# rizar/attention-lvcsr

Measured on NVIDIA H100. Metric: encoder+decoder frames/sec at batch64x1000frx40fb, higher is better.
Workload: dtype f32

## Files before the change

attention-lvcsr_b200/_lib.py:

```python
import ctypes as C
import os

_HERE = os.path.dirname(os.path.abspath(__file__))
LIB_PATH = os.environ.get("LVSR_B200_LIB") or os.path.join(_HERE, "csrc", "liblvsr_b200.so")

LVSR_MAX_LAYERS = 8
NORMALIZERS = {"softmax": 0, "logistic": 1, "relu": 2}
ACTIVATIONS = {"maxout": 0, "relu": 1, "tanh": 2, "identity": 3}
PRIORS = {"expanding": 0, "window_around_mean": 1, "window_around_median": 2}
ATTENTION_TYPES = {"content_and_conv": 0, "content": 1}
PLAN_SLOTS = ("ran", "kernel", "cs", "grid", "nisl", "nrg", "ncg", "nc1", "nc2", "nc3", "tc_cap", "wh_rows", "red_alias",
              "att_cs", "max_clusters")
PLAN_KERNELS = ("stepwise", "dec_scan", "dec_scan<COMPACT>", "dec_content")
ENC_PLAN_SLOTS = ("proj", "kpad", "bigru", "tape", "rb", "cs", "clusters", "resident", "waves", "T", "bwd_cs", "wgrad",
                  "wgrad_splits", "wgrad_kpad", "dx")
ENC_PATHS = (None, "tc", "ffma")
ENC_BIGRU_KERNELS = (None, "ffma", "mma")


class LvsrConfig(C.Structure):
    _fields_ = [
        ("num_features", C.c_int32),
        ("num_layers", C.c_int32),
        ("dims_bidir", C.c_int32 * LVSR_MAX_LAYERS),
        ("subsample", C.c_int32 * LVSR_MAX_LAYERS),
        ("dim_dec", C.c_int32),
        ("dim_matcher", C.c_int32),
        ("conv_n", C.c_int32),
        ("conv_num_filters", C.c_int32),
        ("num_phonemes", C.c_int32),
        ("dim_feedback", C.c_int32),
        ("post_merge_dim", C.c_int32),
        ("maxout_pieces", C.c_int32),
        ("post_merge_activation", C.c_int32),
        ("use_states_for_readout", C.c_int32),
        ("energy_normalizer", C.c_int32),
        ("prior_type", C.c_int32),
        ("prior_initial_begin", C.c_double),
        ("prior_initial_end", C.c_double),
        ("prior_min_speed", C.c_double),
        ("prior_max_speed", C.c_double),
        ("prior_before", C.c_double),
        ("prior_after", C.c_double),
        ("one_of_n_feedback", C.c_int32),
        ("attention_type", C.c_int32),
    ]


class LvsrTrainConfig(C.Structure):
    _fields_ = [("gradient_threshold", C.c_float), ("use_momentum", C.c_int32), ("scale", C.c_float),
                ("momentum", C.c_float), ("use_adadelta", C.c_int32), ("decay_rate", C.c_float),
                ("epsilon", C.c_float), ("max_norm", C.c_float), ("burn_in_steps", C.c_int32), ("decay", C.c_float)]


LM_MAX_STATES = 7


class LvsrLmFusion(C.Structure):
    _fields_ = [("weight", C.c_double), ("am_beta", C.c_double), ("no_transition_cost", C.c_double),
                ("normalize_am_weights", C.c_int32), ("normalize_lm_weights", C.c_int32),
                ("normalize_tot_weights", C.c_int32)]


_P = C.c_void_p
_I = C.c_int32
VALIDATE_FN = C.CFUNCTYPE(C.c_int32, _P, C.c_int32, C.POINTER(C.c_int64), C.c_int32)
SIGNATURES = {
    "lvsr_last_error": (C.c_char_p, []),
    "lvsr_version": (C.c_int, []),
    "lvsr_model_create": (C.c_int, [C.POINTER(LvsrConfig), C.POINTER(_P)]),
    "lvsr_model_destroy": (C.c_int, [_P]),
    "lvsr_model_num_params": (C.c_int, [_P]),
    "lvsr_model_param_name": (C.c_char_p, [_P, C.c_int]),
    "lvsr_model_param_shape": (C.c_int, [_P, C.c_int, C.POINTER(C.c_int64), C.POINTER(C.c_int32)]),
    "lvsr_model_set_param": (C.c_int, [_P, C.c_char_p, _P, C.c_int64]),
    "lvsr_model_get_param": (C.c_int, [_P, C.c_char_p, _P, C.c_int64]),
    "lvsr_model_flat_size": (C.c_int64, [_P]),
    "lvsr_model_param_offset": (C.c_int, [_P, C.c_int, C.POINTER(C.c_int64), C.POINTER(C.c_int64)]),
    "lvsr_model_flat_params": (C.c_void_p, [_P]),
    "lvsr_model_finalize": (C.c_int, [_P]),
    "lvsr_model_status": (C.c_int, [_P, C.POINTER(C.c_int32), C.POINTER(C.c_int64)]),
    "lvsr_model_decoder_plan": (C.c_int, [_P, C.POINTER(C.c_int32)]),
    "lvsr_model_encoder_plan": (C.c_int, [_P, _I, C.POINTER(C.c_int32)]),
    "lvsr_encoded_length": (C.c_int, [_P, _I]),
    "lvsr_encoded_dim": (C.c_int, [_P]),
    "lvsr_encoder_forward": (C.c_int, [_P, _P, _P, _I, _I, _P, _P, _P]),
    "lvsr_preprocess": (C.c_int, [_P, _P, _I, _I, _P, _P]),
    "lvsr_cost_matrix": (C.c_int, [_P, _P, _P, _I, _I, _P, _P, _I, _P, _P, _P, _P, _P, _P]),
    "lvsr_initial_states": (C.c_int, [_P, _I, _I, _P, _P, _P, _P, _P, _P, _P]),
    "lvsr_logprobs": (C.c_int, [_P, _P, _P, _P, _I, _I, _P, _I, _P, _P, _P, _P, _P]),
    "lvsr_next_states": (C.c_int, [_P, _P, _P, _P, _I, _I, _P, _I, _P, _P, _P, _P, _P, _P, _P, _P, _P, _P]),
    "lvsr_beam_search_many": (C.c_int, [_P, _P, _P, _P, _I, _I, _P, _P, _I, _I, _I, C.c_double, C.c_double, _I, VALIDATE_FN,
                                        _P, C.POINTER(_P), _P]),
    "lvsr_search_result_count": (C.c_int, [_P, _I]),
    "lvsr_search_result_length": (C.c_int, [_P, _I, _I]),
    "lvsr_search_result_get": (C.c_int, [_P, _I, _I, _P, _P]),
    "lvsr_search_result_destroy": (C.c_int, [_P]),
    "lvsr_model_set_lm": (C.c_int, [_P, _I, _I, _P, C.c_int64, _P, _P, _P, C.POINTER(LvsrLmFusion)]),
    "lvsr_model_clear_lm": (C.c_int, [_P]),
    "lvsr_lm_initial_states": (C.c_int, [_P, _I, _P, _P, _P, _P]),
    "lvsr_lm_next_states": (C.c_int, [_P, _I, _P, _P, _P, _P, _P, _P, _P]),
    "lvsr_recognizer_cost_host": (C.c_int, [_P, _P, _P, _P, _P, _I, _I, _I, _P, _P]),
    "lvsr_train_cost_and_grads": (C.c_int, [_P, _P, _P, _P, _P, _I, _I, _I, C.c_float, _P, _P, _P]),
    "lvsr_train_apply_updates": (C.c_int, [_P, _P, C.c_float, C.POINTER(LvsrTrainConfig), _P]),
    "lvsr_train_gradient_norm": (C.c_int, [_P, C.POINTER(C.c_float)]),
    "lvsr_train_reset": (C.c_int, [_P]),
    "lvsr_launch_count": (C.c_int64, [C.c_int]),
    "lvsr_profile_enable": (C.c_int, [C.c_int]),
    "lvsr_profile_read": (C.c_int, [C.c_char_p, C.POINTER(C.c_double), C.POINTER(C.c_int64)]),
}

_lib = None


def load():
    global _lib
    if _lib is not None:
        return _lib
    if not os.path.exists(LIB_PATH):
        raise RuntimeError(
            "%s is missing: build it with `python -c 'import __graft_entry__ as g; g.build()'` "
            "(attention-lvcsr_b200 has no CPU or PyTorch fallback)" % LIB_PATH)
    lib = C.CDLL(LIB_PATH)
    for name, (res, args) in SIGNATURES.items():
        fn = getattr(lib, name)
        fn.restype = res
        fn.argtypes = args
    _lib = lib
    return lib


def check(rc):
    if rc != 0:
        msg = load().lvsr_last_error()
        raise RuntimeError("lvsr_b200: " + (msg.decode("utf-8", "replace") if msg else "error %d" % rc))
```

attention-lvcsr_b200/csrc/api.cu:

```cuda
#include "lvsr_b200.h"

#include <stdarg.h>
#include <stdlib.h>

#include <algorithm>
#include <map>
#include <string>
#include <vector>

#include "model.h"

namespace lvsr {

thread_local std::string g_last_error;
long long g_launch_count = 0;

int set_error(const char* fmt, ...) {
  char buf[1024];
  va_list ap;
  va_start(ap, fmt);
  vsnprintf(buf, sizeof(buf), fmt, ap);
  va_end(ap);
  g_last_error = buf;
  return 1;
}

struct ProfEntry { std::string cls; cudaEvent_t a, b; };
static bool g_prof_on = false;
static std::vector<ProfEntry> g_prof;

ProfScope::ProfScope(const char* kernel_class, cudaStream_t stream) : slot(-1), st(stream) {
  if (!g_prof_on) return;
  ProfEntry e;
  e.cls = kernel_class;
  if (cudaEventCreate(&e.a) != cudaSuccess || cudaEventCreate(&e.b) != cudaSuccess) return;
  cudaEventRecord(e.a, st);
  g_prof.push_back(e);
  slot = (int)g_prof.size() - 1;
}
ProfScope::~ProfScope() {
  if (slot >= 0) cudaEventRecord(g_prof[slot].b, st);
}

}

using namespace lvsr;

namespace lvsr {

void add_param(lvsr_model* m, const std::string& name, int64_t d0, int64_t d1 = -1) {
  Param p;
  p.name = name;
  p.shape[0] = d0;
  p.shape[1] = d1 > 0 ? d1 : 1;
  p.ndim = d1 > 0 ? 2 : 1;
  p.count = d0 * (d1 > 0 ? d1 : 1);
  p.dev = nullptr;
  m->index[name] = (int)m->params.size();
  m->params.push_back(p);
}


void build_param_table(lvsr_model* m) {
  const lvsr_config& c = m->cfg;
  int din = c.num_features;
  for (int l = 0; l < c.num_layers; ++l) {
    const int D = c.dims_bidir[l];
    for (int dir = 0; dir < 2; ++dir) {
      const std::string b = enc_base(l, dir);
      add_param(m, b + "/gatedrecurrent.state_to_state", D, D);
      add_param(m, b + "/gatedrecurrent.state_to_gates", D, 2 * D);
      add_param(m, b + "/gatedrecurrent.initial_state", D);
      add_param(m, b + "/fork/fork_inputs.b", D);
      add_param(m, b + "/fork/fork_inputs.W", din, D);
      add_param(m, b + "/fork/fork_gate_inputs.b", 2 * D);
      add_param(m, b + "/fork/fork_gate_inputs.W", din, 2 * D);
    }
    din = 2 * D;
  }
  const int E = m->E, C = c.dim_dec, M = c.dim_matcher, K = c.conv_num_filters, w = 2 * c.conv_n + 1;
  const int V = c.num_phonemes, Cfb = c.dim_feedback, Cpm = c.post_merge_dim;
  const std::string g = GEN, t = TR, a = att_base(m);
  if (!c.one_of_n_feedback) add_param(m, g + "/readout/lookupfeedback/lookuptable.W", V + 1, Cfb);
  if (c.use_states_for_readout) add_param(m, g + "/readout/merge/transform_states.W", C, Cpm);
  add_param(m, g + "/readout/merge/transform_weighted_averages.W", E, Cpm);
  add_param(m, g + "/readout/post_merge/bias.b", Cpm);
  add_param(m, g + "/readout/post_merge/mlp/linear_0.b", V);
  add_param(m, g + "/readout/post_merge/mlp/linear_0.W", Cpm / c.maxout_pieces, V);
  add_param(m, g + "/fork/fork_inputs.b", C);
  add_param(m, g + "/fork/fork_inputs.W", Cfb, C);
  add_param(m, g + "/fork/fork_gate_inputs.b", 2 * C);
  add_param(m, g + "/fork/fork_gate_inputs.W", Cfb, 2 * C);
  add_param(m, t + "/transition.state_to_state", C, C);
  add_param(m, t + "/transition.state_to_gates", C, 2 * C);
  add_param(m, t + "/transition.initial_state", C);
  add_param(m, a + "/state_trans/transform_states.W", C, M);
  add_param(m, a + "/preprocess.b", M);
  add_param(m, a + "/preprocess.W", E, M);
  if (c.energy_normalizer != LVSR_NORM_SOFTMAX) add_param(m, a + "/energy_comp/linear.b", 1);
  add_param(m, a + "/energy_comp/linear.W", M, 1);
  if (!content_attention(m)) {
    add_param(m, a + "/handler.W", K, M);
    add_param(m, a + "/conv1d.filters", K, w);
  }
  add_param(m, t + "/distribute/fork_inputs.W", E, C);
  add_param(m, t + "/distribute/fork_gate_inputs.W", E, 2 * C);
}

int copy_cols(float* dst, int ld_dst, int col0, const float* src, int rows, int cols, cudaStream_t s) {
  LVSR_CUDA_OK(cudaMemcpy2DAsync(dst + col0, (size_t)ld_dst * sizeof(float), src, (size_t)cols * sizeof(float),
                                 (size_t)cols * sizeof(float), rows, cudaMemcpyDeviceToDevice, s));
  return 0;
}



struct Segments {
  const int* seg_start = nullptr; int nseg = 0; const int* seg_len = nullptr; const int* row_seg = nullptr;
};
int glimpses(lvsr_model* m, const float* H, const float* P, const float* maskH, int Tp, int U,
             const int* row_utt, int R, const float* states, const float* w_prev, const long long* step,
             long long step_offset, float* w_out, float* e_out, float* ctx, cudaStream_t st, Segments sg = Segments()) {
  const lvsr_config& c = m->cfg;
  Arena& ws = m->ws;
  float* q = ws.f32((size_t)R * c.dim_matcher);
  int* win = ws.i32((size_t)2 * std::max(1, sg.nseg));
  float* lohi = ws.f32((size_t)2 * R);
  LVSR_CHECK(q && win && lohi, "out of device memory (workspace)");
  DenseArgs d = {};
  d.X1 = states; d.K1 = c.dim_dec; d.W1 = m->P(att_base(m) + "/state_trans/transform_states.W");
  d.R = R; d.N = c.dim_matcher; d.mode = DENSE_PLAIN; d.out = q;
  if (int rc = dense_step(d, st)) return rc;
  WindowArgs wa = {};
  wa.weights = w_prev; wa.step = step; wa.step_offset = step_offset; wa.R = R; wa.Tp = Tp;
  wa.prior = prior_of(c); wa.win = win; wa.lohi = lohi;
  wa.seg_start = sg.seg_start; wa.nseg = sg.nseg; wa.seg_len = sg.seg_len;
  if (int rc = attention_window(wa, st)) return rc;
  AttStepArgs a = {};
  a.P = P; a.H = H; a.maskH = maskH; a.row_utt = row_utt; a.q = q; a.w_prev = w_prev; a.win = win; a.lohi = lohi;
  a.row_seg = sg.seg_start ? sg.row_seg : nullptr;
  a.filt = m->P(att_base(m) + "/conv1d.filters");
  a.Wh = m->P(att_base(m) + "/handler.W");
  a.v = m->P(att_base(m) + "/energy_comp/linear.W");
  a.v_bias = m->v_bias;
  a.w_out = w_out; a.e_out = e_out; a.ctx = ctx;
  a.R = R; a.U = U; a.Tp = Tp; a.M = c.dim_matcher; a.E = m->E; a.K = c.conv_num_filters; a.n = c.conv_n;
  a.normalizer = c.energy_normalizer;
  return attention_step(a, !content_attention(m), &m->att_cs, st);
}

int transition(lvsr_model* m, int R, const float* states, const float* ctx, const long long* outputs,
               const float* rmask, float* next_states, cudaStream_t st) {
  const lvsr_config& c = m->cfg;
  Arena& ws = m->ws;
  const int C = c.dim_dec;
  float* z = ws.f32((size_t)R * C);
  float* hr = ws.f32((size_t)R * C);
  float* ai = ws.f32((size_t)R * C);
  LVSR_CHECK(z && hr && ai, "out of device memory (workspace)");
  DenseArgs g = {};
  g.X1 = ctx; g.K1 = m->E; g.W1 = m->Wd_cat;
  g.X2 = states; g.K2 = C; g.W2 = m->P(std::string(TR) + "/transition.state_to_gates"); g.N2 = 2 * C;
  g.add = m->FF; g.arow = outputs; g.add_rows = c.num_phonemes + 1; g.R = R; g.N = 3 * C; g.mode = DENSE_GATES;
  g.s = states; g.z = z; g.hr = hr; g.ai = ai; g.C = C;
  if (int rc = dense_step(g, st)) return rc;
  DenseArgs k = {};
  k.X1 = hr; k.K1 = C; k.W1 = m->P(std::string(TR) + "/transition.state_to_state");
  k.add = ai; k.arow = nullptr; k.R = R; k.N = C; k.mode = DENSE_CAND;
  k.s = states; k.z = z; k.rmask = rmask; k.out = next_states; k.C = C;
  return dense_step(k, st);
}

int readout_merged(lvsr_model* m, int R, const float* states, const float* ctx, float* merged, cudaStream_t st) {
  const lvsr_config& c = m->cfg;
  DenseArgs d = {};
  d.X1 = ctx; d.K1 = m->E; d.W1 = m->P(std::string(GEN) + "/readout/merge/transform_weighted_averages.W");
  if (c.use_states_for_readout) {
    d.X2 = states; d.K2 = c.dim_dec; d.W2 = m->P(std::string(GEN) + "/readout/merge/transform_states.W");
    d.N2 = c.post_merge_dim;
  }
  d.R = R; d.N = c.post_merge_dim; d.mode = DENSE_PLAIN; d.out = merged;
  return dense_step(d, st);
}

ReadoutArgs readout_args(lvsr_model* m, int R, const float* merged) {
  const lvsr_config& c = m->cfg;
  ReadoutArgs r = {};
  r.merged = merged;
  r.b_pm = m->P(std::string(GEN) + "/readout/post_merge/bias.b");
  r.Wo = m->P(std::string(GEN) + "/readout/post_merge/mlp/linear_0.W");
  r.bo = m->P(std::string(GEN) + "/readout/post_merge/mlp/linear_0.b");
  r.R = R; r.Cpm = c.post_merge_dim; r.pieces = c.maxout_pieces; r.V = c.num_phonemes; r.act = c.post_merge_activation;
  return r;
}

LmFst lm_fst(lvsr_model* m) {
  LmFst f = {};
  f.off = m->lm_off; f.label = m->lm_label; f.next = m->lm_next; f.weight = m->lm_weight;
  f.start = m->lm_start; f.V = m->cfg.num_phonemes;
  f.no_transition_cost = (float)m->lm_fusion.no_transition_cost;
  f.status = m->lm_status;
  return f;
}

void lm_fuse(const lvsr_model* m, ReadoutArgs& r, const float* lm_add) {
  const lvsr_lm_fusion& u = m->lm_fusion;
  r.lm_add = lm_add;
  r.lm_weight = (float)u.weight; r.am_beta = (float)u.am_beta;
  r.norm_am = u.normalize_am_weights != 0; r.norm_lm = u.normalize_lm_weights != 0;
  r.norm_tot = u.normalize_tot_weights != 0;
}

int lm_report(unsigned status) {
  LVSR_CHECK(status != LVSR_LM_TOO_MANY_STATES, "language model: a hypothesis reached more than %d FST states",
             (int)LVSR_LM_MAX_STATES);
  LVSR_CHECK(status != LVSR_LM_CLOSURE_CAP, "language model: an epsilon closure exceeded 32 FST states");
  LVSR_CHECK(status != LVSR_LM_CYCLE, "language model: the FST has an epsilon cycle");
  LVSR_CHECK(status == 0, "language model: status %u", status);
  return 0;
}

static int lm_sync_status(lvsr_model* m, cudaStream_t st) {
  unsigned h = 0;
  LVSR_CUDA_OK(cudaMemcpyAsync(&h, m->lm_status, sizeof(h), cudaMemcpyDeviceToHost, st));
  LVSR_CUDA_OK(cudaStreamSynchronize(st));
  if (h) LVSR_CUDA_OK(cudaMemset(m->lm_status, 0, sizeof(unsigned)));
  return lm_report(h);
}

size_t encoder_ws_bytes(const lvsr_model* m, int T, int B) {
  size_t total = 0;
  int Tl = T;
  for (int l = 0; l < m->cfg.num_layers; ++l) {
    const int D = m->cfg.dims_bidir[l], k = m->cfg.subsample[l];
    const int Tout = ceil_div(Tl, k);
    total += ((size_t)Tl * B * 6 * D + (size_t)Tout * B * 2 * D) * sizeof(float) + 1024;
    total += (size_t)2 * Tl * B * gemm_tc_kpad(l == 0 ? m->cfg.num_features : 2 * m->cfg.dims_bidir[l - 1]) * sizeof(float) + 1024;
    Tl = Tout;
  }
  return total + (1 << 16);
}
size_t cost_ws_bytes(const lvsr_model* m, int Tp, int B, int L) {
  const lvsr_config& c = m->cfg;
  size_t f = (size_t)Tp * B * c.dim_matcher + (size_t)2 * Tp * B * m->E + (size_t)(L + 1) * B * c.dim_dec + (size_t)L * B * m->E +
             (size_t)4 * B * Tp + (size_t)L * B * c.post_merge_dim + (size_t)B * c.dim_matcher +
             (size_t)L * B * (Tp + c.dim_matcher + c.dim_dec + 1) +
             (size_t)3 * B * c.dim_dec + 4 * B + 64;
  return f * sizeof(float) + (1 << 16);
}



}

extern "C" {

const char* lvsr_last_error(void) { return g_last_error.c_str(); }
int lvsr_version(void) { return 104; }
int64_t lvsr_launch_count(int reset) {
  const int64_t v = g_launch_count;
  if (reset) g_launch_count = 0;
  return v;
}

int lvsr_profile_enable(int on) {
  g_prof_on = on != 0;
  return 0;
}
int lvsr_profile_read(const char* kernel_class, double* total_ms, int64_t* count) {
  LVSR_CHECK(kernel_class && total_ms && count, "null argument");
  LVSR_CUDA_OK(cudaDeviceSynchronize());
  double tot = 0.0;
  int64_t n = 0;
  std::vector<ProfEntry> keep;
  for (auto& e : g_prof) {
    if (e.cls == kernel_class) {
      float ms = 0.f;
      if (cudaEventElapsedTime(&ms, e.a, e.b) == cudaSuccess) { tot += ms; n++; }
      cudaEventDestroy(e.a);
      cudaEventDestroy(e.b);
    } else {
      keep.push_back(e);
    }
  }
  g_prof.swap(keep);
  *total_ms = tot;
  *count = n;
  return 0;
}

int lvsr_model_create(const lvsr_config* cfg, lvsr_model** out) {
  LVSR_CHECK(cfg && out, "null argument");
  LVSR_CHECK(cfg->num_layers >= 1 && cfg->num_layers <= LVSR_MAX_LAYERS, "num_layers %d out of range", cfg->num_layers);
  for (int l = 0; l < cfg->num_layers; ++l) {
    LVSR_CHECK(bigru_supported(cfg->dims_bidir[l]), "encoder dim %d unsupported (128 or 256)", cfg->dims_bidir[l]);
    LVSR_CHECK(cfg->subsample[l] >= 1, "subsample must be >= 1");
  }
  LVSR_CHECK(cfg->dim_dec % 8 == 0 && cfg->post_merge_dim % 8 == 0, "dim_dec and post_merge_dim must be multiples of 8");
  LVSR_CHECK(cfg->dim_matcher == 128 || cfg->dim_matcher == 256 || cfg->dim_matcher == 512,
             "dim_matcher %d unsupported by the attention kernel (128, 256 or 512)", cfg->dim_matcher);
  LVSR_CHECK(cfg->one_of_n_feedback ? cfg->dim_feedback == cfg->num_phonemes + 1 : cfg->dim_feedback % 4 == 0,
             "dim_feedback must be a multiple of 4 (LookupFeedback) or num_phonemes + 1 (OneOfNFeedback)");
  LVSR_CHECK(cfg->maxout_pieces >= 1 && cfg->post_merge_dim % cfg->maxout_pieces == 0, "bad maxout_pieces");
  LVSR_CHECK(cfg->post_merge_activation >= LVSR_ACT_MAXOUT && cfg->post_merge_activation <= LVSR_ACT_IDENTITY,
             "bad post_merge_activation");
  LVSR_CHECK(cfg->post_merge_activation == LVSR_ACT_MAXOUT || cfg->maxout_pieces == 1,
             "maxout_pieces must be 1 unless the activation is Maxout");
  LVSR_CHECK(cfg->attention_type == LVSR_ATT_CONTENT_AND_CONV || cfg->attention_type == LVSR_ATT_CONTENT,
             "attention_type %d unsupported (0: content_and_conv, 1: content)", cfg->attention_type);
  const bool content = cfg->attention_type == LVSR_ATT_CONTENT;
  LVSR_CHECK(content || (cfg->conv_num_filters >= 1 && cfg->conv_num_filters <= 16), "conv_num_filters %d not in [1,16]",
             cfg->conv_num_filters);
  LVSR_CHECK(content || cfg->conv_n >= 1, "conv_n must be >= 1 (got %d)", cfg->conv_n);
  LVSR_CHECK(cfg->num_phonemes >= 1 && cfg->num_phonemes <= 128, "num_phonemes out of range");
  int dev_count = 0;
  LVSR_CUDA_OK(cudaGetDeviceCount(&dev_count));
  LVSR_CHECK(dev_count > 0, "no CUDA device: the GPU path has no CPU fallback");
  lvsr_model* m = new lvsr_model();
  m->cfg = *cfg;
  if (content) {
    lvsr_config& c = m->cfg;
    c.conv_n = c.conv_num_filters = 0;
    c.energy_normalizer = LVSR_NORM_SOFTMAX;
    c.prior_type = LVSR_PRIOR_EXPANDING;
    c.prior_initial_begin = 0.0;
    c.prior_initial_end = 1e30;
    c.prior_min_speed = c.prior_max_speed = 0.0;
    c.prior_before = c.prior_after = 0.0;
  }
  LVSR_CUDA_OK(cudaGetDevice(&m->device));
  m->E = 2 * cfg->dims_bidir[cfg->num_layers - 1];
  build_param_table(m);
  int64_t total = 0;
  for (auto& p : m->params) {
    p.offset = total;
    total += (p.count + 63) & ~(int64_t)63;
  }
  m->flat_count = total;
  {
    cudaError_t e = cudaMalloc(reinterpret_cast<void**>(&m->flat), (size_t)total * sizeof(float));
    if (e != cudaSuccess) {
      lvsr_model_destroy(m);
      return set_error("cudaMalloc(parameters, %lld floats) failed: %s", (long long)total, cudaGetErrorString(e));
    }
    cudaMemset(m->flat, 0, (size_t)total * sizeof(float));
  }
  for (auto& p : m->params) p.dev = m->flat + p.offset;
  if (cudaMalloc(reinterpret_cast<void**>(&m->status), 64) != cudaSuccess) {
    lvsr_model_destroy(m);
    return set_error("cudaMalloc(status) failed");
  }
  cudaMemset(m->status, 0, 64);
  *out = m;
  return 0;
}

int lvsr_model_destroy(lvsr_model* m) {
  if (!m) return 0;
  DeviceGuard device_guard(m);
  cudaDeviceSynchronize();
  if (m->flat) cudaFree(m->flat);
  for (float* p : m->Wcat) if (p) cudaFree(p);
  for (float* p : m->bcat) if (p) cudaFree(p);
  for (float* p : m->Wcat_hi) if (p) cudaFree(p);
  for (float* p : m->Wcat_lo) if (p) cudaFree(p);
  if (m->Wp_hi) cudaFree(m->Wp_hi);
  if (m->Wp_lo) cudaFree(m->Wp_lo);
  if (m->Wd_cat) cudaFree(m->Wd_cat);
  if (m->Wb1) cudaFree(m->Wb1);
  if (m->Wff_cat) cudaFree(m->Wff_cat);
  if (m->bff_cat) cudaFree(m->bff_cat);
  if (m->FF) cudaFree(m->FF);
  if (m->status) cudaFree(m->status);
  if (m->opt_velocity) cudaFree(m->opt_velocity);
  if (m->opt_ms_step) cudaFree(m->opt_ms_step);
  if (m->opt_ms_dx) cudaFree(m->opt_ms_dx);
  if (m->opt_scratch) cudaFree(m->opt_scratch);
  if (m->opt_desc) cudaFree(m->opt_desc);
  lvsr_model_clear_lm(m);
  m->tws.destroy();
  m->ws.destroy();
  delete m;
  return 0;
}

int lvsr_model_status(lvsr_model* m, int32_t* launch_status, int64_t* stepwise_fallbacks) {
  DeviceGuard device_guard(m);
  LVSR_CHECK(m && launch_status, "null argument");
  unsigned hst = 0;
  LVSR_CUDA_OK(cudaMemcpy(&hst, m->status, sizeof(hst), cudaMemcpyDeviceToHost));
  *launch_status = (int32_t)hst;
  if (stepwise_fallbacks) *stepwise_fallbacks = m->dec_fallbacks;
  return 0;
}

int lvsr_model_decoder_plan(const lvsr_model* m, int32_t out[16]) {
  LVSR_CHECK(m && out, "null argument");
  for (int i = 0; i < 16; ++i) out[i] = m->dec_plan[i];
  out[LVSR_PLAN_ATT_CS] = m->att_cs;
  return 0;
}

int lvsr_model_encoder_plan(const lvsr_model* m, int32_t layer, int32_t out[16]) {
  LVSR_CHECK(m && out, "null argument");
  LVSR_CHECK(layer >= -1 && layer < m->cfg.num_layers, "encoder_plan: layer %d outside [-1, %d)", layer, m->cfg.num_layers);
  for (int i = 0; i < 16; ++i) out[i] = layer >= 0 ? m->enc_plan[layer][i] : 0;
  if (layer < 0) {
    out[LVSR_ENC_PROJ] = m->pre_plan[0];
    out[LVSR_ENC_KPAD] = m->pre_plan[1];
  }
  return 0;
}

int lvsr_model_num_params(const lvsr_model* m) { return m ? (int)m->params.size() : 0; }
const char* lvsr_model_param_name(const lvsr_model* m, int i) {
  if (!m || i < 0 || i >= (int)m->params.size()) return nullptr;
  return m->params[i].name.c_str();
}
int lvsr_model_param_shape(const lvsr_model* m, int i, int64_t shape[2], int32_t* ndim) {
  LVSR_CHECK(m && i >= 0 && i < (int)m->params.size(), "bad parameter index %d", i);
  shape[0] = m->params[i].shape[0];
  shape[1] = m->params[i].shape[1];
  *ndim = m->params[i].ndim;
  return 0;
}
int64_t lvsr_model_flat_size(const lvsr_model* m) { return m ? m->flat_count : 0; }
int lvsr_model_param_offset(const lvsr_model* m, int i, int64_t* offset, int64_t* count) {
  LVSR_CHECK(m && offset && i >= 0 && i < (int)m->params.size(), "bad parameter index %d", i);
  *offset = m->params[i].offset;
  if (count) *count = m->params[i].count;
  return 0;
}
float* lvsr_model_flat_params(lvsr_model* m) { return m ? m->flat : nullptr; }
int lvsr_model_set_param(lvsr_model* m, const char* name, const float* host, int64_t count) {
  DeviceGuard device_guard(m);
  LVSR_CHECK(m && name && host, "null argument");
  auto it = m->index.find(name);
  LVSR_CHECK(it != m->index.end(), "unknown parameter '%s'", name);
  Param& p = m->params[it->second];
  LVSR_CHECK(count == p.count, "parameter '%s' expects %lld values, got %lld", name, (long long)p.count, (long long)count);
  LVSR_CUDA_OK(cudaMemcpy(p.dev, host, (size_t)count * sizeof(float), cudaMemcpyHostToDevice));
  m->finalized = false;
  return 0;
}
int lvsr_model_get_param(const lvsr_model* m, const char* name, float* host, int64_t count) {
  DeviceGuard device_guard(m);
  LVSR_CHECK(m && name && host, "null argument");
  auto it = m->index.find(name);
  LVSR_CHECK(it != m->index.end(), "unknown parameter '%s'", name);
  const Param& p = m->params[it->second];
  LVSR_CHECK(count == p.count, "parameter '%s' holds %lld values, asked for %lld", name, (long long)p.count, (long long)count);
  LVSR_CUDA_OK(cudaMemcpy(host, p.dev, (size_t)count * sizeof(float), cudaMemcpyDeviceToHost));
  return 0;
}

int lvsr_model_finalize(lvsr_model* m) {
  DeviceGuard device_guard(m);
  LVSR_CHECK(m, "null model");
  return finalize_on_stream(m, 0, true);
}

int lvsr_model_clear_lm(lvsr_model* m) {
  DeviceGuard device_guard(m);
  LVSR_CHECK(m, "null model");
  if (m->lm_off) {
    LVSR_CUDA_OK(cudaDeviceSynchronize());
    cudaFree(m->lm_off); cudaFree(m->lm_label); cudaFree(m->lm_next); cudaFree(m->lm_weight);
  }
  if (m->lm_status) cudaFree(m->lm_status);
  m->lm_off = nullptr; m->lm_label = m->lm_next = nullptr; m->lm_weight = nullptr; m->lm_status = nullptr;
  return 0;
}

int lvsr_model_set_lm(lvsr_model* m, int32_t num_states, int32_t start, const int64_t* off, int64_t num_arcs,
                      const int32_t* label, const int32_t* next, const float* weight, const lvsr_lm_fusion* fusion) {
  DeviceGuard device_guard(m);
  LVSR_CHECK(m && off && fusion && num_states > 0 && num_arcs >= 0 && (num_arcs == 0 || (label && next && weight)),
             "set_lm: bad arguments");
  LVSR_CHECK(start >= 0 && start < num_states, "set_lm: start state %d outside [0, %d)", start, num_states);
  LVSR_CHECK(off[0] == 0 && off[num_states] == num_arcs, "set_lm: arc offsets must run from 0 to num_arcs");
  const int V = m->cfg.num_phonemes;
  for (int32_t s = 0; s < num_states; ++s) {
    LVSR_CHECK(off[s] <= off[s + 1], "set_lm: arc offsets decrease at state %d", s);
    for (int64_t j = off[s]; j < off[s + 1]; ++j) {
      LVSR_CHECK(label[j] >= 0 && label[j] <= V && next[j] >= 0 && next[j] < num_states,
                 "set_lm: arc %lld of state %d has label %d / next state %d out of range", (long long)j, s, label[j], next[j]);
      LVSR_CHECK(j == off[s] || label[j - 1] < label[j] || (label[j - 1] == label[j] && next[j - 1] <= next[j]),
                 "set_lm: the arcs of state %d are not sorted by (label, next state)", s);
    }
  }
  if (int rc = lvsr_model_clear_lm(m)) return rc;
  const size_t na = (size_t)std::max<int64_t>(num_arcs, 1);
  LVSR_CUDA_OK(cudaMalloc(reinterpret_cast<void**>(&m->lm_status), sizeof(unsigned)));
  LVSR_CUDA_OK(cudaMemset(m->lm_status, 0, sizeof(unsigned)));
  LVSR_CUDA_OK(cudaMalloc(reinterpret_cast<void**>(&m->lm_off), (size_t)(num_states + 1) * sizeof(long long)));
  LVSR_CUDA_OK(cudaMalloc(reinterpret_cast<void**>(&m->lm_label), na * sizeof(int)));
  LVSR_CUDA_OK(cudaMalloc(reinterpret_cast<void**>(&m->lm_next), na * sizeof(int)));
  LVSR_CUDA_OK(cudaMalloc(reinterpret_cast<void**>(&m->lm_weight), na * sizeof(float)));
  LVSR_CUDA_OK(cudaMemcpy(m->lm_off, off, (size_t)(num_states + 1) * sizeof(long long), cudaMemcpyHostToDevice));
  if (num_arcs > 0) {
    LVSR_CUDA_OK(cudaMemcpy(m->lm_label, label, (size_t)num_arcs * sizeof(int), cudaMemcpyHostToDevice));
    LVSR_CUDA_OK(cudaMemcpy(m->lm_next, next, (size_t)num_arcs * sizeof(int), cudaMemcpyHostToDevice));
    LVSR_CUDA_OK(cudaMemcpy(m->lm_weight, weight, (size_t)num_arcs * sizeof(float), cudaMemcpyHostToDevice));
  }
  m->lm_start = start;
  m->lm_fusion = *fusion;
  return 0;
}

int lvsr_lm_initial_states(lvsr_model* m, int32_t R, int32_t* states, double* weights, float* add, void* stream) {
  DeviceGuard device_guard(m);
  LVSR_CHECK(m && lm_attached(m), "lm_initial_states: no language model attached");
  LVSR_CHECK(states && weights && add && R > 0, "lm_initial_states: bad arguments");
  cudaStream_t st = static_cast<cudaStream_t>(stream);
  if (int rc = lm_step(lm_fst(m), R, nullptr, nullptr, nullptr, nullptr, states, weights, add, st)) return rc;
  return lm_sync_status(m, st);
}

int lvsr_lm_next_states(lvsr_model* m, int32_t R, const int32_t* states, const double* weights, const int64_t* outputs,
                        int32_t* next_states, double* next_weights, float* next_add, void* stream) {
  DeviceGuard device_guard(m);
  LVSR_CHECK(m && lm_attached(m), "lm_next_states: no language model attached");
  LVSR_CHECK(states && weights && outputs && next_states && next_weights && next_add && R > 0,
             "lm_next_states: bad arguments");
  cudaStream_t st = static_cast<cudaStream_t>(stream);
  if (int rc = lm_step(lm_fst(m), R, states, weights, nullptr, reinterpret_cast<const long long*>(outputs), next_states,
                       next_weights, next_add, st)) return rc;
  return lm_sync_status(m, st);
}

}

namespace lvsr {
int finalize_on_stream(lvsr_model* m, cudaStream_t st, bool synchronise) {
  const lvsr_config& c = m->cfg;
  if (m->Wcat.empty()) {
    int din = c.num_features;
    for (int l = 0; l < c.num_layers; ++l) {
      const int D = c.dims_bidir[l];
      float *W = nullptr, *b = nullptr;
      LVSR_CUDA_OK(cudaMalloc(reinterpret_cast<void**>(&W), (size_t)din * 6 * D * sizeof(float)));
      LVSR_CUDA_OK(cudaMalloc(reinterpret_cast<void**>(&b), (size_t)6 * D * sizeof(float)));
      m->Wcat.push_back(W);
      m->bcat.push_back(b);
      din = 2 * D;
    }
    const int C = c.dim_dec;
    LVSR_CUDA_OK(cudaMalloc(reinterpret_cast<void**>(&m->Wd_cat), (size_t)m->E * 3 * C * sizeof(float)));
    LVSR_CUDA_OK(cudaMalloc(reinterpret_cast<void**>(&m->Wb1), (size_t)(m->E + C) * 3 * C * sizeof(float)));
    LVSR_CUDA_OK(cudaMalloc(reinterpret_cast<void**>(&m->Wff_cat), (size_t)c.dim_feedback * 3 * C * sizeof(float)));
    LVSR_CUDA_OK(cudaMalloc(reinterpret_cast<void**>(&m->bff_cat), (size_t)3 * C * sizeof(float)));
    LVSR_CUDA_OK(cudaMalloc(reinterpret_cast<void**>(&m->FF), (size_t)(c.num_phonemes + 1) * 3 * C * sizeof(float)));
  }
  int din = c.num_features;
  for (int l = 0; l < c.num_layers; ++l) {
    const int D = c.dims_bidir[l];
    for (int dir = 0; dir < 2; ++dir) {
      const std::string b = enc_base(l, dir);
      const int c0 = dir * 3 * D;
      if (int rc = copy_cols(m->Wcat[l], 6 * D, c0, m->P(b + "/fork/fork_inputs.W"), din, D, st)) return rc;
      if (int rc = copy_cols(m->Wcat[l], 6 * D, c0 + D, m->P(b + "/fork/fork_gate_inputs.W"), din, 2 * D, st)) return rc;
      if (int rc = copy_cols(m->bcat[l], 6 * D, c0, m->P(b + "/fork/fork_inputs.b"), 1, D, st)) return rc;
      if (int rc = copy_cols(m->bcat[l], 6 * D, c0 + D, m->P(b + "/fork/fork_gate_inputs.b"), 1, 2 * D, st)) return rc;
    }
    din = 2 * D;
  }
  const int C = c.dim_dec, Cfb = c.dim_feedback, V = c.num_phonemes;
  const std::string g = GEN, t = TR;
  if (int rc = copy_cols(m->Wd_cat, 3 * C, 0, m->P(t + "/distribute/fork_gate_inputs.W"), m->E, 2 * C, st)) return rc;
  if (int rc = copy_cols(m->Wd_cat, 3 * C, 2 * C, m->P(t + "/distribute/fork_inputs.W"), m->E, C, st)) return rc;
  LVSR_CUDA_OK(cudaMemsetAsync(m->Wb1, 0, (size_t)(m->E + C) * 3 * C * sizeof(float), st));
  if (int rc = copy_cols(m->Wb1, 3 * C, 0, m->Wd_cat, m->E, 3 * C, st)) return rc;
  if (int rc = copy_cols(m->Wb1 + (size_t)m->E * 3 * C, 3 * C, 0, m->P(t + "/transition.state_to_gates"), C, 2 * C, st)) return rc;
  if (int rc = copy_cols(m->Wff_cat, 3 * C, 0, m->P(g + "/fork/fork_gate_inputs.W"), Cfb, 2 * C, st)) return rc;
  if (int rc = copy_cols(m->Wff_cat, 3 * C, 2 * C, m->P(g + "/fork/fork_inputs.W"), Cfb, C, st)) return rc;
  if (int rc = copy_cols(m->bff_cat, 3 * C, 0, m->P(g + "/fork/fork_gate_inputs.b"), 1, 2 * C, st)) return rc;
  if (int rc = copy_cols(m->bff_cat, 3 * C, 2 * C, m->P(g + "/fork/fork_inputs.b"), 1, C, st)) return rc;
  m->use_tc = getenv("LVSR_NO_TC_GEMM") == nullptr;
  if (m->use_tc) {
    if (m->Wcat_hi.empty()) {
      int dk = c.num_features;
      for (int l = 0; l < c.num_layers; ++l) {
        const int D = c.dims_bidir[l];
        float *h = nullptr, *lo = nullptr;
        if (gemm_tc_supported(128, 6 * D, dk)) {
          LVSR_CUDA_OK(cudaMalloc(reinterpret_cast<void**>(&h), (size_t)gemm_tc_kpad(dk) * 6 * D * sizeof(float)));
          LVSR_CUDA_OK(cudaMalloc(reinterpret_cast<void**>(&lo), (size_t)gemm_tc_kpad(dk) * 6 * D * sizeof(float)));
        }
        m->Wcat_hi.push_back(h);
        m->Wcat_lo.push_back(lo);
        dk = 2 * D;
      }
      if (gemm_tc_supported(128, c.dim_matcher, m->E)) {
        LVSR_CUDA_OK(cudaMalloc(reinterpret_cast<void**>(&m->Wp_hi), (size_t)gemm_tc_kpad(m->E) * c.dim_matcher * sizeof(float)));
        LVSR_CUDA_OK(cudaMalloc(reinterpret_cast<void**>(&m->Wp_lo), (size_t)gemm_tc_kpad(m->E) * c.dim_matcher * sizeof(float)));
      }
    }
    int dk = c.num_features;
    for (int l = 0; l < c.num_layers; ++l) {
      const int D = c.dims_bidir[l];
      if (m->Wcat_hi[l])
        if (int rc = split_weight_tf32(m->Wcat[l], dk, 6 * D, m->Wcat_hi[l], m->Wcat_lo[l], st)) return rc;
      dk = 2 * D;
    }
    if (m->Wp_hi)
      if (int rc = split_weight_tf32(m->P(att_base(m) + "/preprocess.W"), m->E, c.dim_matcher, m->Wp_hi, m->Wp_lo, st))
        return rc;
  }
  if (c.one_of_n_feedback) {
    if (int rc = add_bias_rows(m->FF, m->Wff_cat, m->bff_cat, V + 1, 3 * C, st)) return rc;
  } else {
    GemmArgs ff = make_gemm(m->P(g + "/readout/lookupfeedback/lookuptable.W"), V + 1, Cfb, m->Wff_cat, 3 * C,
                            m->bff_cat, m->FF);
    if (int rc = gemm_bias(ff, st)) return rc;
  }
  m->v_bias = 0.f;
  if (c.energy_normalizer != LVSR_NORM_SOFTMAX)
    LVSR_CUDA_OK(cudaMemcpy(&m->v_bias, m->P(att_base(m) + "/energy_comp/linear.b"), sizeof(float),
                            cudaMemcpyDeviceToHost));
  if (synchronise) LVSR_CUDA_OK(cudaStreamSynchronize(st));
  m->finalized = true;
  return 0;
}

int projection_gemm(Arena& ws, const float* A, int M, int K, const float* W, const float* W_hi, const float* W_lo, int N,
                    const float* bias, float* out, cudaStream_t st, int* kpad) {
  if (W_hi && gemm_tc_supported(M, N, K)) {
    float* a_hi = ws.f32((size_t)M * gemm_tc_kpad(K));
    float* a_lo = ws.f32((size_t)M * gemm_tc_kpad(K));
    LVSR_CHECK(a_hi && a_lo, "out of device memory (tf32 split scratch)");
    if (kpad) *kpad = gemm_tc_kpad(K);
    return gemm_tc(A, a_hi, a_lo, M, K, W_hi, W_lo, N, bias, out, N, st);
  }
  if (kpad) *kpad = 0;
  return gemm_bias(make_gemm(A, M, K, W, N, bias, out), st);
}

int run_encoder(lvsr_model* m, Arena& ws, const float* x, const float* mask, int T, int B, float* attended,
                float* attended_mask, LayerTape* tape, cudaStream_t st) {
  const lvsr_config& c = m->cfg;
  const float* cur = x;
  int Tl = T, din = c.num_features;
  long long mstride = B;
  int kcum = 1;
  for (int l = 0; l < c.num_layers; ++l)
    for (int s = LVSR_ENC_PROJ; s <= LVSR_ENC_T; ++s) m->enc_plan[l][s] = 0;
  for (int l = 0; l < c.num_layers; ++l) {
    const int D = c.dims_bidir[l], k = c.subsample[l];
    const int rows = Tl * B, Tout = ceil_div(Tl, k);
    float* pre = ws.f32((size_t)rows * 6 * D);
    float* hext = tape ? ws.f32((size_t)(Tl + 2) * B * 2 * D) : nullptr;
    LVSR_CHECK(pre && (hext || !tape), "out of device memory (encoder pre-activations)");
    const size_t mark = ws.off;
    int32_t* plan = m->enc_plan[l];
    int kpad = 0;
    if (int rc = projection_gemm(ws, cur, rows, din, m->Wcat[l], m->use_tc ? m->Wcat_hi[l] : nullptr,
                                 m->use_tc ? m->Wcat_lo[l] : nullptr, 6 * D, m->bcat[l], pre, st, &kpad))
      return rc;
    plan[LVSR_ENC_PROJ] = kpad ? LVSR_ENC_PATH_TC : LVSR_ENC_PATH_FFMA;
    plan[LVSR_ENC_KPAD] = kpad;
    if (ws.off <= ws.cap) ws.off = mark;
    float* out = (l == c.num_layers - 1) ? attended : ws.f32((size_t)Tout * B * 2 * D);
    LVSR_CHECK(out, "out of device memory (encoder layer output)");
    BiGruArgs a = {};
    a.pre = pre; a.mask = mask; a.mask_tstride = mstride;
    const std::string bf = enc_base(l, 0) + "/gatedrecurrent", bb = enc_base(l, 1) + "/gatedrecurrent";
    a.Wg_f = m->P(bf + ".state_to_gates"); a.Ws_f = m->P(bf + ".state_to_state"); a.h0_f = m->P(bf + ".initial_state");
    a.Wg_b = m->P(bb + ".state_to_gates"); a.Ws_b = m->P(bb + ".state_to_state"); a.h0_b = m->P(bb + ".initial_state");
    a.out = out; a.T = Tl; a.B = B; a.D = D; a.subsample = k;
    if (tape) {
      a.tape = pre; a.hext = hext;
      tape[l] = {cur, pre, hext, out, Tl, Tout, din, D, k, mstride};
    }
    BiGruPlan bp;
    if (int rc = bigru_layer(a, st, &bp)) return rc;
    plan[LVSR_ENC_BIGRU] = bp.kernel;
    plan[LVSR_ENC_TAPE] = tape ? 1 : 0;
    plan[LVSR_ENC_RB] = bp.rb;
    plan[LVSR_ENC_CS] = bp.cs;
    plan[LVSR_ENC_CLUSTERS] = bp.clusters;
    plan[LVSR_ENC_RESIDENT] = bp.resident;
    plan[LVSR_ENC_WAVES] = bp.waves;
    plan[LVSR_ENC_T] = Tl;
    cur = out; Tl = Tout; din = 2 * D; mstride *= k; kcum *= k;
  }
  if (mask) {
    if (int rc = gather_time_subsample(attended_mask, mask, Tl, kcum, B, st)) return rc;
  } else {
    if (int rc = fill_f32(attended_mask, (long long)Tl * B, 1.f, st)) return rc;
  }
  return 0;
}
}

extern "C" {

int lvsr_encoded_length(const lvsr_model* m, int32_t T) {
  if (!m) return 0;
  int t = T;
  for (int l = 0; l < m->cfg.num_layers; ++l) t = ceil_div(t, m->cfg.subsample[l]);
  return t;
}
int lvsr_encoded_dim(const lvsr_model* m) { return m ? m->E : 0; }

int lvsr_encoder_forward(lvsr_model* m, const float* x, const float* mask, int32_t T, int32_t B,
                         float* attended, float* attended_mask, void* stream) {
  DeviceGuard device_guard(m);
  if (int rc = check_ready(m)) return rc;
  LVSR_CHECK(x && attended && attended_mask && T > 0 && B > 0, "encoder_forward: bad arguments");
  cudaStream_t st = static_cast<cudaStream_t>(stream);
  m->ws.reserve(encoder_ws_bytes(m, T, B), st);
  ArenaScope scope(m, st);
  return run_encoder(m, m->ws, x, mask, T, B, attended, attended_mask, nullptr, st);
}

int lvsr_preprocess(lvsr_model* m, const float* attended, int32_t Tp, int32_t U, float* out, void* stream) {
  DeviceGuard device_guard(m);
  if (int rc = check_ready(m)) return rc;
  LVSR_CHECK(attended && out && Tp > 0 && U > 0, "preprocess: bad arguments");
  cudaStream_t st = static_cast<cudaStream_t>(stream);
  ArenaScope scope(m, st);
  int kpad = 0;
  m->pre_plan[0] = m->pre_plan[1] = 0;
  if (int rc = projection_gemm(m->ws, attended, Tp * U, m->E, m->P(att_base(m) + "/preprocess.W"),
                               m->use_tc ? m->Wp_hi : nullptr, m->Wp_lo, m->cfg.dim_matcher,
                               m->P(att_base(m) + "/preprocess.b"), out, st, &kpad))
    return rc;
  m->pre_plan[0] = kpad ? LVSR_ENC_PATH_TC : LVSR_ENC_PATH_FFMA;
  m->pre_plan[1] = kpad;
  return 0;
}

int lvsr_cost_matrix(lvsr_model* m, const float* attended, const float* attended_mask, int32_t Tp, int32_t B,
                     const int64_t* labels, const float* labels_mask, int32_t L, float* costs,
                     float* weights_out, float* energies_out, float* states_out, float* wavg_out, void* stream) {
  DeviceGuard device_guard(m);
  if (int rc = check_ready(m)) return rc;
  LVSR_CHECK(attended && attended_mask && labels && costs && Tp > 0 && B > 0 && L > 0, "cost_matrix: bad arguments");
  cudaStream_t st = static_cast<cudaStream_t>(stream);
  m->ws.reserve(cost_ws_bytes(m, Tp, B, L) + (lm_attached(m) ? (size_t)L * B * m->cfg.num_phonemes * sizeof(float) : 0), st);
  ArenaScope scope(m, st);
  const lvsr_config& c = m->cfg;
  Arena& ws = m->ws;
  const int C = c.dim_dec, E = m->E, M = c.dim_matcher;
  const long long* lab = reinterpret_cast<const long long*>(labels);

  float* P = ws.f32((size_t)Tp * B * M);
  float* s_all = ws.f32((size_t)(L + 1) * B * C);
  float* ctx_all = wavg_out ? wavg_out : ws.f32((size_t)L * B * E);
  float* w0 = ws.f32((size_t)B * Tp);
  float* wpp[2] = {ws.f32((size_t)B * Tp), ws.f32((size_t)B * Tp)};
  float* e_scratch = energies_out ? nullptr : ws.f32((size_t)B * Tp);
  float* merged = ws.f32((size_t)L * B * c.post_merge_dim);
  LVSR_CHECK(P && s_all && ctx_all && w0 && merged && wpp[0] && wpp[1] && (energies_out || e_scratch),
             "out of device memory (decoder workspace)");

  if (int rc = lvsr_preprocess(m, attended, Tp, B, P, stream)) return rc;
  if (int rc = broadcast_rows(s_all, m->P(std::string(TR) + "/transition.initial_state"), B, C, st)) return rc;
  if (int rc = onehot_rows(w0, B, Tp, st)) return rc;
  if (int rc = fill_f32(costs, (long long)L * B, 0.f, st)) return rc;

  bool scanned = false;
  for (int32_t& v : m->dec_plan) v = 0;
  LVSR_CUDA_OK(cudaMemsetAsync(m->status, 0, sizeof(unsigned), st));
  if (getenv("LVSR_NO_DEC_SCAN") == nullptr && !m->force_stepwise) {
    DecScanArgs d = {};
    d.P = P; d.H = attended; d.maskH = attended_mask;
    d.filt = m->P(att_base(m) + "/conv1d.filters");
    d.Wh = m->P(att_base(m) + "/handler.W");
    d.v = m->P(att_base(m) + "/energy_comp/linear.W");
    d.v_bias = m->v_bias;
    d.prior = prior_of(c);
    d.Wb1 = m->Wb1;
    d.Wstate = m->P(std::string(TR) + "/transition.state_to_state");
    d.Ws = m->P(att_base(m) + "/state_trans/transform_states.W");
    d.FF = m->FF;
    d.labels = lab; d.lmask = labels_mask;
    d.s_all = s_all; d.ctx_all = ctx_all; d.w0 = w0;
    d.e_seq = energies_out; d.e_scratch = e_scratch;
    d.status = m->status;
    d.Tp = Tp; d.B = B; d.L = L; d.M = M; d.E = E; d.C = C; d.K = c.conv_num_filters; d.n = c.conv_n;
    d.normalizer = c.energy_normalizer;
    d.V = c.num_phonemes;
    d.w_all = weights_out ? weights_out : ws.f32((size_t)L * B * Tp);
    d.q_all = ws.f32((size_t)L * B * M);
    d.hr_all = ws.f32((size_t)L * B * C);
    d.rowpos_all = ws.f32((size_t)(L + 1) * B);
    LVSR_CHECK(d.w_all && d.q_all && d.hr_all && d.rowpos_all,
               "out of device memory (decoder scan workspace)");
    LVSR_CUDA_OK(cudaMemsetAsync(d.w_all, 0xFF, (size_t)L * B * Tp * sizeof(float), st));
    LVSR_CUDA_OK(cudaMemsetAsync(d.q_all, 0xFF, (size_t)L * B * M * sizeof(float), st));
    LVSR_CUDA_OK(cudaMemsetAsync(d.hr_all, 0xFF, (size_t)L * B * C * sizeof(float), st));
    LVSR_CUDA_OK(cudaMemsetAsync(d.rowpos_all + B, 0xFF, (size_t)L * B * sizeof(float), st));
    LVSR_CUDA_OK(cudaMemsetAsync(d.rowpos_all, 0, (size_t)B * sizeof(float), st));
    LVSR_CUDA_OK(cudaMemsetAsync(s_all + (size_t)B * C, 0xFF, (size_t)L * B * C * sizeof(float), st));
    LVSR_CUDA_OK(cudaMemsetAsync(ctx_all, 0xFF, (size_t)L * B * E * sizeof(float), st));
    const bool trace = getenv("LVSR_DEC_TRACE") != nullptr;
    if (trace) {
      d.trace = reinterpret_cast<unsigned long long*>(ws.i64((size_t)2 * L * 9 + (size_t)L * 12 + (size_t)L * B));
      LVSR_CUDA_OK(cudaMemsetAsync(d.trace, 0, ((size_t)2 * L * 9 + (size_t)L * 12 + (size_t)L * B) * 8, st));
    }
    int supported = 0, grid = 0, max_clusters = 0;
    if (int rc = dec_scan_try(d, !content_attention(m), &supported, &grid, &max_clusters, st)) return rc;
    scanned = supported != 0;
    int32_t* p = m->dec_plan;
    p[LVSR_PLAN_MAX_CLUSTERS] = max_clusters;
    if (scanned) {
      p[LVSR_PLAN_RAN] = 1;
      p[LVSR_PLAN_KERNEL] = content_attention(m) ? LVSR_PLAN_DEC_CONTENT : d.wh_rows != 16 ? LVSR_PLAN_DEC_SCAN_COMPACT
                                                                                            : LVSR_PLAN_DEC_SCAN;
      p[LVSR_PLAN_CS] = d.cs; p[LVSR_PLAN_GRID] = grid; p[LVSR_PLAN_NISL] = d.nisl; p[LVSR_PLAN_NRG] = d.nrg;
      p[LVSR_PLAN_NCG] = d.ncg; p[LVSR_PLAN_NC1] = d.nc1; p[LVSR_PLAN_NC2] = d.nc2; p[LVSR_PLAN_NC3] = d.nc3;
      p[LVSR_PLAN_TC_CAP] = d.tc_cap; p[LVSR_PLAN_WH_ROWS] = d.wh_rows; p[LVSR_PLAN_RED_ALIAS] = d.red_alias;
    }
    if (scanned && getenv("LVSR_DEC_CHECK") != nullptr) {
      LVSR_CUDA_OK(cudaStreamSynchronize(st));
      unsigned hst = 0;
      LVSR_CUDA_OK(cudaMemcpy(&hst, m->status, sizeof(hst), cudaMemcpyDeviceToHost));
      LVSR_CHECK(hst == 0, "LVSR_DEC_CHECK: persistent decoder launch status %u (2 = a value never arrived, "
                 "3 = launched without its cluster shape)", hst);
      struct { const char* name; const float* p; size_t n; } bufs[] = {
          {"weights", d.w_all, (size_t)L * B * Tp}, {"queries", d.q_all, (size_t)L * B * M},
          {"reset-gated states", d.hr_all, (size_t)L * B * C}, {"states", s_all, (size_t)(L + 1) * B * C},
          {"weighted averages", ctx_all, (size_t)L * B * E},
          {"row positions", d.rowpos_all, c.prior_type == LVSR_PRIOR_EXPANDING ? (size_t)B : (size_t)(L + 1) * B}};
      for (auto& b : bufs) {
        long long left = 0;
        if (int rc = count_sentinels(b.p, (long long)b.n, &left, st)) return rc;
        LVSR_CHECK(left == 0, "LVSR_DEC_CHECK: %lld sentinel words left in the %s buffer", left, b.name);
      }
    }
    if (trace && scanned) {
      std::vector<unsigned long long> h((size_t)2 * L * 9 + (size_t)L * 12 + (size_t)L * B);
      LVSR_CUDA_OK(cudaMemcpyAsync(h.data(), d.trace, h.size() * 8, cudaMemcpyDeviceToHost, st));
      LVSR_CUDA_OK(cudaStreamSynchronize(st));
      const char* names[8] = {"A", "syncA", "B1", "sync1", "B2", "sync2", "B3", "sync3"};
      for (int slot = 0; slot < 2; ++slot) {
        double sum[8] = {0};
        int n = 0;
        for (int i = 1; i + 1 < L; ++i, ++n)
          for (int j = 0; j < 8; ++j) sum[j] += (double)(h[((size_t)slot * L + i) * 9 + j + 1] - h[((size_t)slot * L + i) * 9 + j]);
        fprintf(stderr, "[dec_scan trace] CTA %s:", slot == 0 ? "first" : "last");
        for (int j = 0; j < 8; ++j) fprintf(stderr, " %s=%.2fus", names[j], n ? sum[j] / n * 1e-3 : 0.0);
        fprintf(stderr, "\n");
      }
      {
        const char* an[7] = {"stage", "conv", "energy", "stats", "ctx", "exchange", "combine"};
        double sum[7] = {0};
        int n = 0;
        for (int i = 1; i + 1 < L; ++i, ++n)
          for (int j = 0; j < 7; ++j)
            sum[j] += (double)(h[(size_t)2 * L * 9 + (size_t)i * 8 + j + 1] - h[(size_t)2 * L * 9 + (size_t)i * 8 + j]);
        fprintf(stderr, "[dec_scan trace] attention row 0:");
        for (int j = 0; j < 7; ++j) fprintf(stderr, " %s=%.2fus", an[j], n ? sum[j] / n * 1e-3 : 0.0);
        fprintf(stderr, "\n");
      }
      {
        double sum[4] = {0};
        int n = 0;
        for (int i = 1; i + 1 < L; ++i, ++n) {
          const unsigned long long* b = &h[(size_t)0 * L * 9 + (size_t)i * 9];
          const unsigned long long* t = &h[(size_t)2 * L * 9 + (size_t)L * 8 + (size_t)i * 4];
          sum[0] += (double)(t[0] - b[2]); sum[1] += (double)(t[1] - t[0]);
          sum[2] += (double)(t[2] - t[1]); sum[3] += (double)(b[3] - t[2]);
        }
        {
          fprintf(stderr, "[dec_scan trace] end of attention vs row 0 (us):");
          for (int r = 0; r < B; ++r) {
            double acc = 0;
            for (int i = 1; i + 1 < L; ++i) {
              const unsigned long long* e = &h[(size_t)2 * L * 9 + (size_t)L * 12 + (size_t)i * B];
              acc += (double)((long long)e[r] - (long long)e[0]);
            }
            fprintf(stderr, " %.1f", acc / (L - 2) * 1e-3);
          }
          fprintf(stderr, "\n");
        }
        fprintf(stderr, "[dec_scan trace] gate tile: wait_x=%.2fus products=%.2fus sums=%.2fus epilogue=%.2fus\n",
                n ? sum[0] / n * 1e-3 : 0.0, n ? sum[1] / n * 1e-3 : 0.0, n ? sum[2] / n * 1e-3 : 0.0,
                n ? sum[3] / n * 1e-3 : 0.0);
      }
    }
  }
  const float* w_prev = w0;
  for (int i = 0; i < L && !scanned; ++i) {
    float* w_i = weights_out ? weights_out + (size_t)i * B * Tp : wpp[i & 1];
    float* e_i = energies_out ? energies_out + (size_t)i * B * Tp : e_scratch;
    float* ctx_i = ctx_all + (size_t)i * B * E;
    const float* s_i = s_all + (size_t)i * B * C;
    const size_t mark = ws.off;
    if (int rc = glimpses(m, attended, P, attended_mask, Tp, B, nullptr, B, s_i, w_prev, nullptr, i, w_i, e_i, ctx_i, st)) return rc;
    if (int rc = transition(m, B, s_i, ctx_i, lab + (size_t)i * B, labels_mask ? labels_mask + (size_t)i * B : nullptr,
                            s_all + (size_t)(i + 1) * B * C, st)) return rc;
    if (ws.off <= ws.cap) ws.off = mark;
    w_prev = w_i;
  }
  float* lm_add = nullptr;
  if (lm_attached(m)) {
    lm_add = ws.f32((size_t)L * B * c.num_phonemes);
    LVSR_CHECK(lm_add, "out of device memory (language model costs)");
    if (int rc = lm_path(lm_fst(m), L, B, lab, labels_mask, lm_add, st)) return rc;
    if (int rc = lm_sync_status(m, st)) return rc;
  }
  {
    const int R = L * B;
    const std::string g = GEN;
    bool acc = false;
    if (c.use_states_for_readout) {
      GemmArgs a = make_gemm(s_all, R, C, m->P(g + "/readout/merge/transform_states.W"), c.post_merge_dim, nullptr, merged);
      if (int rc = gemm_bias(a, st)) return rc;
      acc = true;
    }
    GemmArgs b = make_gemm(ctx_all, R, E, m->P(g + "/readout/merge/transform_weighted_averages.W"), c.post_merge_dim,
                           nullptr, merged, acc);
    if (int rc = gemm_bias(b, st)) return rc;
    ReadoutArgs r = readout_args(m, R, merged);
    r.labels = lab; r.lmask = labels_mask; r.costs_picked = costs;
    r.poison = scanned ? m->status : nullptr;
    if (lm_add) lm_fuse(m, r, lm_add);
    if (int rc = readout_costs(r, st)) return rc;
  }
  if (states_out)
    LVSR_CUDA_OK(cudaMemcpyAsync(states_out, s_all, (size_t)L * B * C * sizeof(float), cudaMemcpyDeviceToDevice, st));
  return 0;
}

int lvsr_initial_states(lvsr_model* m, int32_t Tp, int32_t R, float* states, int64_t* outputs, float* wavg,
                        float* weights, float* energies, int64_t* step, void* stream) {
  DeviceGuard device_guard(m);
  if (int rc = check_ready(m)) return rc;
  LVSR_CHECK(states && outputs && wavg && weights && energies && step && Tp > 0 && R > 0, "initial_states: bad arguments");
  cudaStream_t st = static_cast<cudaStream_t>(stream);
  const lvsr_config& c = m->cfg;
  if (int rc = broadcast_rows(states, m->P(std::string(TR) + "/transition.initial_state"), R, c.dim_dec, st)) return rc;
  if (int rc = fill_i64(reinterpret_cast<long long*>(outputs), R, c.num_phonemes, st)) return rc;
  if (int rc = fill_f32(wavg, (long long)R * m->E, 0.f, st)) return rc;
  if (content_attention(m)) {
    if (int rc = fill_f32(weights, (long long)R * Tp, 0.f, st)) return rc;
    if (int rc = fill_f32(energies, (long long)R * Tp, 0.f, st)) return rc;
  } else {
    if (int rc = onehot_rows(weights, R, Tp, st)) return rc;
    if (int rc = onehot_rows(energies, R, Tp, st)) return rc;
  }
  return fill_i64(reinterpret_cast<long long*>(step), R, 0, st);
}

int lvsr_logprobs(lvsr_model* m, const float* attended, const float* preprocessed, const float* attended_mask,
                  int32_t Tp, int32_t U, const int32_t* row_utt, int32_t R, const float* states,
                  const float* weights, const int64_t* step, float* out, void* stream) {
  DeviceGuard device_guard(m);
  if (int rc = check_ready(m)) return rc;
  LVSR_CHECK(attended && attended_mask && states && weights && step && out && Tp > 0 && U > 0 && R > 0,
             "logprobs: bad arguments");
  LVSR_CHECK(row_utt || U == R, "logprobs: without row_utt the contexts must be replicated (U == R)");
  cudaStream_t st = static_cast<cudaStream_t>(stream);
  ArenaScope scope(m, st);
  const lvsr_config& c = m->cfg;
  Arena& ws = m->ws;
  const float* P = preprocessed;
  if (!P) {
    float* Pb = ws.f32((size_t)Tp * U * c.dim_matcher);
    LVSR_CHECK(Pb, "out of device memory (preprocessed)");
    if (int rc = lvsr_preprocess(m, attended, Tp, U, Pb, stream)) return rc;
    P = Pb;
  }
  float* w_tmp = ws.f32((size_t)R * Tp);
  float* e_tmp = ws.f32((size_t)R * Tp);
  float* ctx = ws.f32((size_t)R * m->E);
  float* merged = ws.f32((size_t)R * c.post_merge_dim);
  LVSR_CHECK(w_tmp && e_tmp && ctx && merged, "out of device memory (logprobs workspace)");
  if (int rc = glimpses(m, attended, P, attended_mask, Tp, U, row_utt, R, states, weights,
                        reinterpret_cast<const long long*>(step), 0, w_tmp, e_tmp, ctx, st)) return rc;
  if (int rc = readout_merged(m, R, states, ctx, merged, st)) return rc;
  ReadoutArgs r = readout_args(m, R, merged);
  r.costs_all = out;
  return readout_costs(r, st);
}

int lvsr_next_states(lvsr_model* m, const float* attended, const float* preprocessed, const float* attended_mask,
                     int32_t Tp, int32_t U, const int32_t* row_utt, int32_t R, const float* states,
                     const float* weights, const int64_t* step, const int64_t* outputs, float* next_states,
                     float* next_wavg, float* next_weights, float* next_energies, int64_t* next_step, void* stream) {
  DeviceGuard device_guard(m);
  if (int rc = check_ready(m)) return rc;
  LVSR_CHECK(attended && attended_mask && states && weights && step && outputs && next_states && next_wavg &&
                 next_weights && next_energies && next_step && Tp > 0 && U > 0 && R > 0,
             "next_states: bad arguments");
  LVSR_CHECK(row_utt || U == R, "next_states: without row_utt the contexts must be replicated (U == R)");
  cudaStream_t st = static_cast<cudaStream_t>(stream);
  ArenaScope scope(m, st);
  const lvsr_config& c = m->cfg;
  Arena& ws = m->ws;
  const float* P = preprocessed;
  if (!P) {
    float* Pb = ws.f32((size_t)Tp * U * c.dim_matcher);
    LVSR_CHECK(Pb, "out of device memory (preprocessed)");
    if (int rc = lvsr_preprocess(m, attended, Tp, U, Pb, stream)) return rc;
    P = Pb;
  }
  if (int rc = glimpses(m, attended, P, attended_mask, Tp, U, row_utt, R, states, weights,
                        reinterpret_cast<const long long*>(step), 0, next_weights, next_energies, next_wavg, st)) return rc;
  if (int rc = transition(m, R, states, next_wavg, reinterpret_cast<const long long*>(outputs), nullptr, next_states, st)) return rc;
  return add_i64(reinterpret_cast<long long*>(next_step), reinterpret_cast<const long long*>(step), R, 1, st);
}

}

namespace lvsr {

int search_expand(lvsr_model* m, const float* attended, const float* preprocessed, const float* attended_mask, int Tp,
                  int U, const int* utt_len, const int* row_utt, const int* row_seg, const int* seg_start, int nseg,
                  int R, const float* states, const float* weights, const long long* step, const float* cost_so_far,
                  const float* lm_add, int k, float* wavg, float* new_weights, float* new_energies, int* top_parent,
                  int* top_symbol, float* top_cost, int* top_count, cudaStream_t st) {
  ArenaScope scope(m, st);
  const lvsr_config& c = m->cfg;
  Arena& ws = m->ws;
  float* merged = ws.f32((size_t)R * c.post_merge_dim);
  float* neglogp = ws.f32((size_t)R * c.num_phonemes);
  LVSR_CHECK(merged && neglogp, "out of device memory (search workspace)");
  Segments sg;
  sg.seg_start = seg_start; sg.nseg = nseg; sg.seg_len = utt_len; sg.row_seg = row_seg;
  if (int rc = glimpses(m, attended, preprocessed, attended_mask, Tp, U, row_utt, R, states, weights, step, 0,
                        new_weights, new_energies, wavg, st, sg)) return rc;
  if (int rc = readout_merged(m, R, states, wavg, merged, st)) return rc;
  ReadoutArgs r = readout_args(m, R, merged);
  r.costs_all = neglogp;
  if (lm_add) lm_fuse(m, r, lm_add);
  if (int rc = readout_costs(r, st)) return rc;
  return segment_topk(neglogp, cost_so_far, seg_start, nseg, c.num_phonemes, k, top_parent, top_symbol, top_cost, top_count, st);
}

int search_advance(lvsr_model* m, const float* attended, const float* preprocessed, const float* attended_mask, int Tp,
                   int U, const int* utt_len, int Rn, const int* parent, const long long* symbols, const int* row_utt,
                   const int* row_seg, const int* seg_start, int nseg, const float* states, const float* weights,
                   const long long* step, const float* wavg, const float* new_weights, const float* new_energies,
                   float* n_states, float* n_wavg, float* n_weights, float* n_energies, long long* n_step,
                   cudaStream_t st) {
  ArenaScope scope(m, st);
  const lvsr_config& c = m->cfg;
  Arena& ws = m->ws;
  const int C = c.dim_dec, E = m->E;
  float* s_sel = ws.f32((size_t)Rn * C);
  LVSR_CHECK(s_sel, "out of device memory (search workspace)");
  if (int rc = gather_rows(s_sel, states, parent, Rn, C, st)) return rc;
  if (c.prior_type == LVSR_PRIOR_EXPANDING) {
    if (int rc = gather_rows(n_wavg, wavg, parent, Rn, E, st)) return rc;
    if (int rc = gather_rows(n_weights, new_weights, parent, Rn, Tp, st)) return rc;
    if (int rc = gather_rows(n_energies, new_energies, parent, Rn, Tp, st)) return rc;
  } else {
    float* w_sel = ws.f32((size_t)Rn * Tp);
    long long* st_sel = ws.i64((size_t)Rn);
    LVSR_CHECK(w_sel && st_sel, "out of device memory (search workspace)");
    if (int rc = gather_rows(w_sel, weights, parent, Rn, Tp, st)) return rc;
    if (int rc = gather_i64(st_sel, step, parent, Rn, 0, st)) return rc;
    Segments sg;
    sg.seg_start = seg_start; sg.nseg = nseg; sg.seg_len = utt_len; sg.row_seg = row_seg;
    if (int rc = glimpses(m, attended, preprocessed, attended_mask, Tp, U, row_utt, Rn, s_sel, w_sel, st_sel, 0, n_weights,
                          n_energies, n_wavg, st, sg)) return rc;
  }
  if (int rc = transition(m, Rn, s_sel, n_wavg, symbols, nullptr, n_states, st)) return rc;
  return gather_i64(n_step, step, parent, Rn, 1, st);
}

}

extern "C" {

int lvsr_recognizer_cost_host(lvsr_model* m, const float* x_h, const float* mask_h, const int64_t* labels_h,
                              const float* lmask_h, int32_t T, int32_t B, int32_t L, float* costs_h, void* stream) {
  DeviceGuard device_guard(m);
  if (int rc = check_ready(m)) return rc;
  LVSR_CHECK(x_h && labels_h && costs_h && T > 0 && B > 0 && L > 0, "recognizer_cost_host: bad arguments");
  for (long long i = 0; i < (long long)L * B; ++i)
    LVSR_CHECK(labels_h[i] >= 0 && labels_h[i] < m->cfg.num_phonemes,
               "recognizer_cost_host: label %lld at [%lld, %lld] outside [0, %d)", (long long)labels_h[i], i / B, i % B,
               m->cfg.num_phonemes);
  cudaStream_t st = static_cast<cudaStream_t>(stream);
  int rc = 0;
  {
    const int F = m->cfg.num_features, Tp = lvsr_encoded_length(m, T), E = m->E;
    m->ws.reserve(encoder_ws_bytes(m, T, B) + cost_ws_bytes(m, Tp, B, L) +
                      ((size_t)T * B * (F + 1) + (size_t)3 * L * B + (size_t)Tp * B * (E + 1)) * sizeof(float) + (1 << 16),
                  st);
    ArenaScope scope(m, st);
    Arena& ws = m->ws;
    float* x = ws.f32((size_t)T * B * F);
    float* mask = mask_h ? ws.f32((size_t)T * B) : nullptr;
    long long* lab = ws.i64((size_t)L * B);
    float* lmask = lmask_h ? ws.f32((size_t)L * B) : nullptr;
    float* att = ws.f32((size_t)Tp * B * E);
    float* attm = ws.f32((size_t)Tp * B);
    float* costs = ws.f32((size_t)L * B);
    LVSR_CHECK(x && lab && att && attm && costs && (!mask_h || mask) && (!lmask_h || lmask), "out of device memory (host call)");
    LVSR_CUDA_OK(cudaMemcpyAsync(x, x_h, (size_t)T * B * F * sizeof(float), cudaMemcpyHostToDevice, st));
    if (mask) LVSR_CUDA_OK(cudaMemcpyAsync(mask, mask_h, (size_t)T * B * sizeof(float), cudaMemcpyHostToDevice, st));
    LVSR_CUDA_OK(cudaMemcpyAsync(lab, labels_h, (size_t)L * B * sizeof(long long), cudaMemcpyHostToDevice, st));
    if (lmask) LVSR_CUDA_OK(cudaMemcpyAsync(lmask, lmask_h, (size_t)L * B * sizeof(float), cudaMemcpyHostToDevice, st));
    rc = lvsr_encoder_forward(m, x, mask, T, B, att, attm, stream);
    if (!rc) rc = lvsr_cost_matrix(m, att, attm, Tp, B, reinterpret_cast<const int64_t*>(lab), lmask, L, costs,
                                   nullptr, nullptr, nullptr, nullptr, stream);
    if (!rc) {
      unsigned hst = 0;
      LVSR_CUDA_OK(cudaMemcpyAsync(costs_h, costs, (size_t)L * B * sizeof(float), cudaMemcpyDeviceToHost, st));
      LVSR_CUDA_OK(cudaMemcpyAsync(&hst, m->status, sizeof(hst), cudaMemcpyDeviceToHost, st));
      LVSR_CUDA_OK(cudaStreamSynchronize(st));
      if (hst != 0) {
        if (m->dec_fallbacks++ == 0)
          fprintf(stderr, "[lvsr_b200] persistent decoder launch failed (status %u); re-running on the step-wise kernels\n", hst);
        m->force_stepwise = true;
        rc = lvsr_cost_matrix(m, att, attm, Tp, B, reinterpret_cast<const int64_t*>(lab), lmask, L, costs,
                              nullptr, nullptr, nullptr, nullptr, stream);
        m->force_stepwise = false;
        if (!rc) {
          LVSR_CUDA_OK(cudaMemcpyAsync(costs_h, costs, (size_t)L * B * sizeof(float), cudaMemcpyDeviceToHost, st));
          LVSR_CUDA_OK(cudaStreamSynchronize(st));
        }
      }
    }
  }
  return rc;
}

}
```

attention-lvcsr_b200/csrc/gemm_tc.cu:

```cuda
#include <cuda.h>

#include "kernels.h"

namespace lvsr {

namespace {

constexpr int TC_BM = 128, TC_BN = 128, TC_BK = 32;
constexpr int TC_THREADS = 384;
constexpr int TC_STAGES = 3;
constexpr uint32_t TC_TILE_BYTES = TC_BM * TC_BK * sizeof(float);
constexpr uint32_t TC_STAGE_BYTES = 4 * TC_TILE_BYTES;
constexpr size_t TC_SMEM = (size_t)TC_STAGES * TC_STAGE_BYTES + 1024  + 256 ;

__device__ __forceinline__ uint32_t smem_addr(const void* p) { return static_cast<uint32_t>(__cvta_generic_to_shared(p)); }

__device__ __forceinline__ void bar_init(uint32_t bar, uint32_t count) {
  asm volatile("mbarrier.init.shared::cta.b64 [%0], %1;\n" ::"r"(bar), "r"(count) : "memory");
}
__device__ __forceinline__ void bar_expect_tx(uint32_t bar, uint32_t bytes) {
  asm volatile("mbarrier.arrive.expect_tx.shared::cta.b64 _, [%0], %1;\n" ::"r"(bar), "r"(bytes) : "memory");
}
__device__ __forceinline__ void bar_arrive(uint32_t bar) {
  asm volatile("mbarrier.arrive.shared::cta.b64 _, [%0];\n" ::"r"(bar) : "memory");
}
__device__ __forceinline__ void bar_wait(uint32_t bar, uint32_t parity) {
  uint32_t ok = 0;
  unsigned long long spins = 0;
  while (true) {
    asm volatile(
        "{\n\t.reg .pred p;\n\t"
        "mbarrier.try_wait.parity.shared::cta.b64 p, [%1], %2;\n\t"
        "selp.u32 %0, 1, 0, p;\n\t}\n"
        : "=r"(ok)
        : "r"(bar), "r"(parity)
        : "memory");
    if (ok) break;
    if (++spins > (1ull << 24)) __trap();
  }
}
__device__ __forceinline__ void tma_load_2d(uint32_t dst, const CUtensorMap* map, int x, int y, uint32_t bar) {
  asm volatile(
      "cp.async.bulk.tensor.2d.shared::cluster.global.mbarrier::complete_tx::bytes [%0], [%1, {%2, %3}], [%4];\n" ::"r"(dst),
      "l"(reinterpret_cast<uint64_t>(map)), "r"(x), "r"(y), "r"(bar)
      : "memory");
}

__device__ __forceinline__ uint64_t make_smem_desc(uint32_t saddr) {
  uint64_t d = 0;
  d |= (uint64_t)((saddr >> 4) & 0x3FFF);
  d |= (uint64_t)1 << 16;
  d |= (uint64_t)(1024 >> 4) << 32;
  d |= (uint64_t)1 << 62;
  return d;
}
__device__ __forceinline__ void wgmma_fence() { asm volatile("wgmma.fence.sync.aligned;\n" ::: "memory"); }
__device__ __forceinline__ void wgmma_commit() { asm volatile("wgmma.commit_group.sync.aligned;\n" ::: "memory"); }
template <int N>
__device__ __forceinline__ void wgmma_wait() { asm volatile("wgmma.wait_group.sync.aligned %0;\n" ::"n"(N) : "memory"); }
template <int N>
__device__ __forceinline__ void acc_fence(float (&d)[N]) {
#pragma unroll
  for (int i = 0; i < N; ++i) asm volatile("" : "+f"(d[i])::"memory");
}

#define LVSR_ACC8(d, i) \
  "+f"(d[i]), "+f"(d[i + 1]), "+f"(d[i + 2]), "+f"(d[i + 3]), "+f"(d[i + 4]), "+f"(d[i + 5]), "+f"(d[i + 6]), "+f"(d[i + 7])
__device__ __forceinline__ void wgmma_tf32_n128(float (&d)[64], uint64_t desc_a, uint64_t desc_b, uint32_t scale_d) {
  asm volatile(
      "{\n\t.reg .pred p;\n\t"
      "setp.ne.b32 p, %66, 0;\n\t"
      "wgmma.mma_async.sync.aligned.m64n128k8.f32.tf32.tf32 {"
      "%0, %1, %2, %3, %4, %5, %6, %7, %8, %9, %10, %11, %12, %13, %14, %15, "
      "%16, %17, %18, %19, %20, %21, %22, %23, %24, %25, %26, %27, %28, %29, %30, %31, "
      "%32, %33, %34, %35, %36, %37, %38, %39, %40, %41, %42, %43, %44, %45, %46, %47, "
      "%48, %49, %50, %51, %52, %53, %54, %55, %56, %57, %58, %59, %60, %61, %62, %63"
      "}, %64, %65, p, 1, 1;\n\t}\n"
      : LVSR_ACC8(d, 0), LVSR_ACC8(d, 8), LVSR_ACC8(d, 16), LVSR_ACC8(d, 24),
        LVSR_ACC8(d, 32), LVSR_ACC8(d, 40), LVSR_ACC8(d, 48), LVSR_ACC8(d, 56)
      : "l"(desc_a), "l"(desc_b), "r"(scale_d));
}
#undef LVSR_ACC8

struct TcGemmParams {
  float* C;
  const float* bias;
  int M, N, K, ldc;
  int kb_per_split;
  long long c_split_stride;
};

__global__ void __launch_bounds__(TC_THREADS, 1)
gemm_tc_kernel(const __grid_constant__ CUtensorMap map_a_hi, const __grid_constant__ CUtensorMap map_a_lo,
               const __grid_constant__ CUtensorMap map_b_hi, const __grid_constant__ CUtensorMap map_b_lo,
               TcGemmParams p) {
  extern __shared__ uint8_t smem_raw[];
  uint8_t* tiles = reinterpret_cast<uint8_t*>((reinterpret_cast<uintptr_t>(smem_raw) + 1023) & ~(uintptr_t)1023);
  constexpr int NACC = TC_BN / 2;
  unsigned long long* bars = reinterpret_cast<unsigned long long*>(tiles + (size_t)TC_STAGES * TC_STAGE_BYTES);

  const int wg = threadIdx.x >> 7, t = threadIdx.x & 127;
  const int n0 = blockIdx.x * TC_BN, m0 = blockIdx.y * TC_BM;
  const int kb0 = blockIdx.z * p.kb_per_split;
  const int nkb = min(p.kb_per_split, p.K / TC_BK - kb0);
  p.C += (long long)blockIdx.z * p.c_split_stride;

  if (threadIdx.x == 0) {
    for (int s = 0; s < TC_STAGES; ++s) {
      bar_init(smem_addr(&bars[s]), 1);
      bar_init(smem_addr(&bars[TC_STAGES + s]), 2);
    }
    asm volatile("fence.mbarrier_init.release.cluster;\n" ::: "memory");
  }
  __syncthreads();

  if (wg == 0) {
    if (t == 0) {
      for (int kb = 0; kb < nkb; ++kb) {
        const int s = kb % TC_STAGES;
        const uint32_t ph = (uint32_t)((kb / TC_STAGES) & 1);
        bar_wait(smem_addr(&bars[TC_STAGES + s]), ph ^ 1u);
        const uint32_t full = smem_addr(&bars[s]);
        bar_expect_tx(full, TC_STAGE_BYTES);
        const uint32_t base = smem_addr(tiles + (size_t)s * TC_STAGE_BYTES);
        tma_load_2d(base + 0 * TC_TILE_BYTES, &map_a_hi, (kb0 + kb) * TC_BK, m0, full);
        tma_load_2d(base + 1 * TC_TILE_BYTES, &map_a_lo, (kb0 + kb) * TC_BK, m0, full);
        tma_load_2d(base + 2 * TC_TILE_BYTES, &map_b_hi, (kb0 + kb) * TC_BK, n0, full);
        tma_load_2d(base + 3 * TC_TILE_BYTES, &map_b_lo, (kb0 + kb) * TC_BK, n0, full);
      }
    }
    return;
  }

  const uint32_t a_off = (uint32_t)(wg - 1) * 64 * 128;
  float acc[NACC];
#pragma unroll
  for (int i = 0; i < NACC; ++i) acc[i] = 0.f;
  for (int kb = 0; kb < nkb; ++kb) {
    const int s = kb % TC_STAGES;
    bar_wait(smem_addr(&bars[s]), (uint32_t)((kb / TC_STAGES) & 1));
    const uint32_t base = smem_addr(tiles + (size_t)s * TC_STAGE_BYTES);
    const uint64_t da_hi = make_smem_desc(base + 0 * TC_TILE_BYTES + a_off), da_lo = make_smem_desc(base + 1 * TC_TILE_BYTES + a_off);
    const uint64_t db_hi = make_smem_desc(base + 2 * TC_TILE_BYTES), db_lo = make_smem_desc(base + 3 * TC_TILE_BYTES);
    wgmma_fence();
#pragma unroll
    for (int k = 0; k < 4; ++k) {
      const uint64_t adv = (uint64_t)(k * 2);
      wgmma_tf32_n128(acc, da_lo + adv, db_hi + adv, 1u);
      wgmma_tf32_n128(acc, da_hi + adv, db_lo + adv, 1u);
      wgmma_tf32_n128(acc, da_hi + adv, db_hi + adv, 1u);
    }
    wgmma_commit();
    wgmma_wait<1>();
    acc_fence(acc);
    if (kb > 0 && t == 0) bar_arrive(smem_addr(&bars[TC_STAGES + (kb - 1) % TC_STAGES]));
  }
  wgmma_wait<0>();
  acc_fence(acc);

  const int warp = t >> 5, lane = t & 31;
  const int r0 = m0 + (wg - 1) * 64 + warp * 16 + (lane >> 2);
  const int cbase = n0 + 2 * (lane & 3);
#pragma unroll
  for (int j = 0; j < TC_BN / 8; ++j) {
    const int col = cbase + 8 * j;
    float2 b = make_float2(0.f, 0.f);
    if (p.bias) b = __ldg(reinterpret_cast<const float2*>(p.bias + col));
#pragma unroll
    for (int h = 0; h < 2; ++h) {
      const int row = r0 + 8 * h;
      const float x = acc[4 * j + 2 * h], y = acc[4 * j + 2 * h + 1];
      if (row < p.M) *reinterpret_cast<float2*>(p.C + (long long)row * p.ldc + col) = make_float2(x + b.x, y + b.y);
    }
  }
}

__global__ void split_tf32_kernel(const float4* __restrict__ x, float4* __restrict__ hi, float4* __restrict__ lo,
                                  long long n4) {
  for (long long i = blockIdx.x * (long long)blockDim.x + threadIdx.x; i < n4; i += (long long)gridDim.x * blockDim.x) {
    const float4 v = x[i];
    float4 h, l;
    auto split = [](float a, float& ah, float& al) {
      ah = __uint_as_float(__float_as_uint(a) & 0xFFFFE000u);
      const float r = a - ah;
      uint32_t t;
      asm("cvt.rna.tf32.f32 %0, %1;\n" : "=r"(t) : "f"(r));
      al = __uint_as_float(t);
    };
    split(v.x, h.x, l.x); split(v.y, h.y, l.y); split(v.z, h.z, l.z); split(v.w, h.w, l.w);
    hi[i] = h;
    lo[i] = l;
  }
}

__global__ void transpose_split_kernel(const float* __restrict__ W, float* __restrict__ hi, float* __restrict__ lo,
                                       int K, int N, int Kpad, int ldw) {
  __shared__ float tile[32][33];
  const int k0 = blockIdx.y * 32, n0 = blockIdx.x * 32;
  for (int i = threadIdx.y; i < 32; i += blockDim.y) {
    const int k = k0 + i, n = n0 + threadIdx.x;
    tile[i][threadIdx.x] = (k < K && n < N) ? W[(long long)k * ldw + n] : 0.f;
  }
  __syncthreads();
  for (int i = threadIdx.y; i < 32; i += blockDim.y) {
    const int n = n0 + i, k = k0 + threadIdx.x;
    if (n < N && k < Kpad) {
      const float a = tile[threadIdx.x][i];
      const float ah = __uint_as_float(__float_as_uint(a) & 0xFFFFE000u);
      uint32_t t;
      asm("cvt.rna.tf32.f32 %0, %1;\n" : "=r"(t) : "f"(a - ah));
      hi[(long long)n * Kpad + k] = ah;
      lo[(long long)n * Kpad + k] = __uint_as_float(t);
    }
  }
}

__global__ void split_pad_tf32_kernel(const float* __restrict__ x, float* __restrict__ hi, float* __restrict__ lo,
                                      long long M, int K, int Kpad) {
  const long long total = M * Kpad;
  for (long long i = blockIdx.x * (long long)blockDim.x + threadIdx.x; i < total; i += (long long)gridDim.x * blockDim.x) {
    const long long r = i / Kpad;
    const int k = (int)(i % Kpad);
    const float a = k < K ? x[r * K + k] : 0.f;
    const float ah = __uint_as_float(__float_as_uint(a) & 0xFFFFE000u);
    uint32_t t;
    asm("cvt.rna.tf32.f32 %0, %1;\n" : "=r"(t) : "f"(a - ah));
    hi[i] = ah;
    lo[i] = __uint_as_float(t);
  }
}

typedef CUresult (*EncodeTiledFn)(CUtensorMap*, CUtensorMapDataType, cuuint32_t, void*, const cuuint64_t*, const cuuint64_t*,
                                  const cuuint32_t*, const cuuint32_t*, CUtensorMapInterleave, CUtensorMapSwizzle,
                                  CUtensorMapL2promotion, CUtensorMapFloatOOBfill);
EncodeTiledFn g_encode = nullptr;

int get_encode() {
  if (g_encode) return 0;
  void* fn = nullptr;
  cudaDriverEntryPointQueryResult qres;
  LVSR_CUDA_OK(cudaGetDriverEntryPoint("cuTensorMapEncodeTiled", &fn, cudaEnableDefault, &qres));
  LVSR_CHECK(fn != nullptr && qres == cudaDriverEntryPointSuccess, "cuTensorMapEncodeTiled not available");
  g_encode = reinterpret_cast<EncodeTiledFn>(fn);
  return 0;
}

int make_map(CUtensorMap* map, const float* ptr, long long rows, int K, int box_rows = TC_BM) {
  cuuint64_t dims[2] = {(cuuint64_t)K, (cuuint64_t)rows};
  cuuint64_t strides[1] = {(cuuint64_t)K * sizeof(float)};
  cuuint32_t box[2] = {(cuuint32_t)TC_BK, (cuuint32_t)box_rows};
  cuuint32_t estr[2] = {1, 1};
  CUresult r = g_encode(map, CU_TENSOR_MAP_DATA_TYPE_FLOAT32, 2, const_cast<float*>(ptr), dims, strides, box, estr,
                        CU_TENSOR_MAP_INTERLEAVE_NONE, CU_TENSOR_MAP_SWIZZLE_128B, CU_TENSOR_MAP_L2_PROMOTION_L2_128B,
                        CU_TENSOR_MAP_FLOAT_OOB_FILL_NONE);
  LVSR_CHECK(r == CUDA_SUCCESS, "cuTensorMapEncodeTiled failed (%d)", (int)r);
  return 0;
}

}

int gemm_tc_kpad(int K) { return ceil_div(K, TC_BK) * TC_BK; }

bool gemm_tc_supported(int M, int N, int K) {
  return M >= 1 && N % TC_BN == 0 && K >= 4 && K % 4 == 0;
}

int split_weight_tf32(const float* W, int K, int N, float* Wt_hi, float* Wt_lo, cudaStream_t stream) {
  const int Kpad = gemm_tc_kpad(K);
  dim3 grid(ceil_div(N, 32), ceil_div(Kpad, 32)), block(32, 8);
  transpose_split_kernel<<<grid, block, 0, stream>>>(W, Wt_hi, Wt_lo, K, N, Kpad, N);
  LVSR_LAUNCH_CHECK();
  return 0;
}

int transpose_split_tf32(const float* W, int K, int N, int ldw, float* hi, float* lo, cudaStream_t stream) {
  const int Kpad = gemm_tc_kpad(K);
  dim3 grid(ceil_div(N, 32), ceil_div(Kpad, 32)), block(32, 8);
  LVSR_CHECK(grid.y <= 65535, "transpose_split: too many rows (%d)", K);
  transpose_split_kernel<<<grid, block, 0, stream>>>(W, hi, lo, K, N, Kpad, ldw);
  LVSR_LAUNCH_CHECK();
  return 0;
}

int split_tf32(const float* x, float* hi, float* lo, long long n, cudaStream_t stream) {
  const long long n4 = n / 4;
  split_tf32_kernel<<<(int)std::min<long long>(4096, (n4 + 255) / 256), 256, 0, stream>>>(
      reinterpret_cast<const float4*>(x), reinterpret_cast<float4*>(hi), reinterpret_cast<float4*>(lo), n4);
  LVSR_LAUNCH_CHECK();
  return 0;
}

int gemm_tc_splits_launched(int Kpad, int splits) {
  const int total_kb = Kpad / TC_BK;
  splits = std::max(1, std::min(splits, total_kb));
  return ceil_div(total_kb, ceil_div(total_kb, splits));
}

int gemm_tc_presplit(const float* A_hi, const float* A_lo, int M, const float* B_hi, const float* B_lo, int N, int Kpad,
                     const float* bias, float* C, int ldc, int splits, long long split_stride, cudaStream_t stream) {
  ProfScope prof("gemm", stream);
  LVSR_CHECK(M >= 1 && N % TC_BN == 0 && Kpad % TC_BK == 0 && Kpad >= TC_BK && splits >= 1, "gemm_tc_presplit: unsupported shape M=%d N=%d K=%d", M, N, Kpad);
  if (int rc = get_encode()) return rc;
  CUtensorMap ma_hi, ma_lo, mb_hi, mb_lo;
  if (int rc = make_map(&ma_hi, A_hi, M, Kpad)) return rc;
  if (int rc = make_map(&ma_lo, A_lo, M, Kpad)) return rc;
  if (int rc = make_map(&mb_hi, B_hi, N, Kpad)) return rc;
  if (int rc = make_map(&mb_lo, B_lo, N, Kpad)) return rc;
  static bool configured[LVSR_MAX_DEVICES] = {false};
  const int dev = current_device();
  if (!configured[dev]) {
    LVSR_CUDA_OK(cudaFuncSetAttribute(gemm_tc_kernel, cudaFuncAttributeMaxDynamicSharedMemorySize, (int)TC_SMEM));
    configured[dev] = true;
  }
  const int total_kb = Kpad / TC_BK;
  splits = std::min(splits, total_kb);
  TcGemmParams p;
  p.C = C; p.bias = bias; p.M = M; p.N = N; p.K = Kpad; p.ldc = ldc;
  p.kb_per_split = ceil_div(total_kb, splits);
  p.c_split_stride = split_stride;
  dim3 grid(N / TC_BN, ceil_div(M, TC_BM), ceil_div(total_kb, p.kb_per_split));
  gemm_tc_kernel<<<grid, TC_THREADS, TC_SMEM, stream>>>(ma_hi, ma_lo, mb_hi, mb_lo, p);
  LVSR_LAUNCH_CHECK();
  return 0;
}

int gemm_tc(const float* A, float* A_hi, float* A_lo, int M, int K, const float* Wt_hi, const float* Wt_lo, int N,
            const float* bias, float* C, int ldc, cudaStream_t stream) {
  LVSR_CHECK(gemm_tc_supported(M, N, K), "gemm_tc: unsupported shape M=%d N=%d K=%d", M, N, K);
  if (int rc = get_encode()) return rc;
  const int Kpad = gemm_tc_kpad(K);
  if (Kpad == K) {
    const long long n4 = (long long)M * K / 4;
    split_tf32_kernel<<<(int)std::min<long long>(4096, (n4 + 255) / 256), 256, 0, stream>>>(
        reinterpret_cast<const float4*>(A), reinterpret_cast<float4*>(A_hi), reinterpret_cast<float4*>(A_lo), n4);
  } else {
    const long long n = (long long)M * Kpad;
    split_pad_tf32_kernel<<<(int)std::min<long long>(4096, (n + 255) / 256), 256, 0, stream>>>(A, A_hi, A_lo, M, K, Kpad);
  }
  LVSR_LAUNCH_CHECK();
  return gemm_tc_presplit(A_hi, A_lo, M, Wt_hi, Wt_lo, N, Kpad, bias, C, ldc, 1, 0, stream);
}

}
```

attention-lvcsr_b200/csrc/kernels.h:

```cpp
#pragma once
#include "common.cuh"

namespace lvsr {

struct GemmArgs {
  const float* A;
  int M, K;
  int rows_per_block;
  long long block_stride;
  int lda;
  const float* W;
  int N, ldw;
  const float* bias;
  float* C;
  int ldc;
  int accumulate;
};
int gemm_bias(const GemmArgs& g, cudaStream_t stream);

inline GemmArgs make_gemm(const float* A, int M, int K, const float* W, int N, const float* bias,
                          float* C, bool accumulate = false) {
  GemmArgs g;
  g.A = A; g.M = M; g.K = K; g.rows_per_block = M > 0 ? M : 1; g.block_stride = 0; g.lda = K;
  g.W = W; g.N = N; g.ldw = N; g.bias = bias; g.C = C; g.ldc = N; g.accumulate = accumulate ? 1 : 0;
  return g;
}

bool gemm_tc_supported(int M, int N, int K);
int gemm_tc_kpad(int K);
int split_weight_tf32(const float* W, int K, int N, float* Wt_hi, float* Wt_lo, cudaStream_t stream);
int transpose_split_tf32(const float* W, int K, int N, int ldw, float* hi, float* lo, cudaStream_t stream);
int split_tf32(const float* x, float* hi, float* lo, long long n, cudaStream_t stream);
int gemm_tc_presplit(const float* A_hi, const float* A_lo, int M, const float* B_hi, const float* B_lo, int N, int Kpad,
                     const float* bias, float* C, int ldc, int splits, long long split_stride, cudaStream_t stream);
int gemm_tc_splits_launched(int Kpad, int splits);
int gemm_tc(const float* A, float* A_hi, float* A_lo, int M, int K, const float* Wt_hi, const float* Wt_lo, int N,
            const float* bias, float* C, int ldc, cudaStream_t stream);

struct BiGruArgs {
  const float* pre;
  const float* mask;
  long long mask_tstride;
  const float *Wg_f, *Ws_f, *h0_f;
  const float *Wg_b, *Ws_b, *h0_b;
  float* out;
  int T, B, D, subsample;
  float* tape;
  float* hext;
};
bool bigru_supported(int D);
struct BiGruPlan { int kernel, rb, cs, clusters, resident, waves; };
int bigru_layer(const BiGruArgs& a, cudaStream_t stream, BiGruPlan* plan = nullptr);

struct BiGruBwdArgs {
  float* tape;
  const float* hext;
  const float* mask;
  long long mask_tstride;
  const float* dout;
  const float *Wg_f, *Ws_f, *Wg_b, *Ws_b;
  float* hr_out;
  float* dh0;
  int T, B, D, subsample;
};
int bigru_layer_backward(const BiGruBwdArgs& a, cudaStream_t stream, int* cs_out = nullptr);

struct PriorParams {
  int type;
  double initial_begin, initial_end, min_speed, max_speed, before, after;
};

struct WindowArgs {
  const float* weights;
  const long long* step;
  long long step_offset;
  int R, Tp;
  PriorParams prior;
  int* win;
  float* lohi;
  const int* seg_start;
  int nseg;
  const int* seg_len;
};
int attention_window(const WindowArgs& a, cudaStream_t stream);

struct AttStepArgs {
  const float* P;
  const float* H;
  const float* maskH;
  const int* row_utt;
  const float* q;
  const float* w_prev;
  const int* win;
  const int* row_seg;
  const float* lohi;
  const float* filt;
  const float* Wh;
  const float* v;
  float v_bias;
  float* w_out;
  float* e_out;
  float* ctx;
  int R, U, Tp, M, E, K, n, normalizer;
};
int attention_step(const AttStepArgs& a, bool location, int* cs_out, cudaStream_t stream);
int attention_max_cluster();

enum { DENSE_PLAIN = 0, DENSE_GATES = 1, DENSE_CAND = 2 };
struct DenseArgs {
  const float* X1; int K1; const float* W1;
  const float* X2; int K2; const float* W2; int N2;
  const float* add;
  const long long* arow;
  long long add_rows;
  int R, N, mode;
  float* out;
  const float* s;
  float* z; float* hr; float* ai;
  const float* rmask;
  int C;
};
int dense_step(const DenseArgs& a, cudaStream_t stream);

struct ReadoutArgs {
  const float* merged;
  const float* b_pm;
  const float* Wo;
  const float* bo;
  int R, Cpm, pieces, V, act;
  const long long* labels;
  const float* lmask;
  float* costs_all;
  float* costs_picked;
  const unsigned* poison;
  const float* lm_add;
  float lm_weight, am_beta;
  int norm_am, norm_lm, norm_tot;
};
int readout_costs(const ReadoutArgs& a, cudaStream_t stream);

enum { LVSR_LM_TOO_MANY_STATES = 1, LVSR_LM_CLOSURE_CAP = 2, LVSR_LM_CYCLE = 3 };
struct LmFst {
  const long long* off;
  const int* label;
  const int* next;
  const float* weight;
  int start, V;
  float no_transition_cost;
  unsigned* status;
};
int lm_step(const LmFst& f, int R, const int* src_states, const double* src_weights, const int* parent,
            const long long* symbols, int* states_out, double* weights_out, float* add_out, cudaStream_t stream);
int lm_path(const LmFst& f, int L, int B, const long long* labels, const float* lmask, float* add, cudaStream_t stream);
int lm_gather(int* states, double* weights, float* add, const int* src_states, const double* src_weights,
              const float* src_add, const int* idx, int Rn, int V, cudaStream_t stream);

struct DecScanArgs {
  const float *P, *H, *maskH;
  const float *filt, *Wh, *v;
  float v_bias;
  PriorParams prior;
  const float* Wb1;
  const float* Wstate;
  const float* Ws;
  const float* FF;
  const long long* labels;
  const float* lmask;
  float* s_all;
  float* ctx_all;
  const float* w0;
  float* w_all;
  float* e_seq;
  float* e_scratch;
  float* q_all;
  float* hr_all;
  float* rowpos_all;
  unsigned long long* trace;
  unsigned* status;
  int Tp, B, L, M, E, C, K, n, normalizer;
  int V;
  int cs, tc_cap, nrg, nc1, nc2, nc3;
  int nisl, ncg;
  int wh_rows;
  int red_alias;
};
int dec_scan_try(DecScanArgs& a, bool location, int* supported, int* grid, int* max_clusters, cudaStream_t stream);

int fill_f32(float* p, long long n, float v, cudaStream_t stream);
int fill_i64(long long* p, long long n, long long v, cudaStream_t stream);
int broadcast_rows(float* dst, const float* src, int R, int N, cudaStream_t stream);
int onehot_rows(float* dst, int R, int N, cudaStream_t stream);
int count_sentinels(const float* p, long long n, long long* host_count, cudaStream_t stream);
int gather_rows(float* dst, const float* src, const int* idx, int Rn, int N, cudaStream_t stream);
int gather_i64(long long* dst, const long long* src, const int* idx, int Rn, long long inc, cudaStream_t stream);
int segment_topk(const float* neglogp, const float* cost_so_far, const int* seg_start, int nseg, int V, int k,
                 int* top_parent, int* top_symbol, float* top_cost, int* top_count, cudaStream_t stream);
int add_bias_rows(float* dst, const float* src, const float* bias, int R, int N, cudaStream_t stream);
int add_i64(long long* dst, const long long* src, int n, long long inc, cudaStream_t stream);
int gather_time_subsample(float* dst, const float* src, int Tout, int k, long long row_elems,
                          cudaStream_t stream);

}
```

attention-lvcsr_b200/csrc/model.h:

```cpp
#pragma once
#include <map>
#include <string>
#include <vector>

#include "kernels.h"
#include "lvsr_b200.h"

namespace lvsr {

struct Arena {
  char* base = nullptr;
  size_t cap = 0, off = 0, overflow_bytes = 0;
  int depth = 0;
  std::vector<void*> overflow;
  cudaStream_t last_stream = nullptr;
  bool used = false;
  void bind_stream(cudaStream_t st) {
    if (depth == 0 && used && st != last_stream) cudaStreamSynchronize(last_stream);
    last_stream = st;
    used = true;
  }

  void* alloc(size_t bytes) {
    bytes = (bytes + 255) & ~(size_t)255;
    if (off + bytes <= cap) {
      void* p = base + off;
      off += bytes;
      return p;
    }
    void* p = nullptr;
    if (cudaMalloc(&p, bytes) != cudaSuccess) return nullptr;
    overflow.push_back(p);
    overflow_bytes += bytes;
    return p;
  }
  float* f32(size_t n) { return static_cast<float*>(alloc(n * sizeof(float))); }
  long long* i64(size_t n) { return static_cast<long long*>(alloc(n * sizeof(long long))); }
  int* i32(size_t n) { return static_cast<int*>(alloc(n * sizeof(int))); }

  void reserve(size_t bytes, cudaStream_t stream) {
    if (off != 0 || bytes <= cap) return;
    if (cudaStreamSynchronize(stream) != cudaSuccess) return;
    if (base) cudaFree(base - shift);
    base = nullptr;
    cap = 0;
    shift = getenv("LVSR_WS_SHIFT_KB") ? (size_t)atoll(getenv("LVSR_WS_SHIFT_KB")) * 1024 : 0;
    if (cudaMalloc(reinterpret_cast<void**>(&base), bytes + shift) == cudaSuccess) { cap = bytes; base += shift; }
    else cudaGetLastError();
  }
  size_t shift = 0;
  void enter() { depth++; }
  int leave(cudaStream_t stream) {
    depth--;
    if (depth > 0) return 0;
    const size_t used = off;
    off = 0;
    if (!overflow.empty()) {
      if (cudaStreamSynchronize(stream) != cudaSuccess) return 1;
      for (void* p : overflow) cudaFree(p);
      overflow.clear();
      if (base) cudaFree(base - shift);
      base = nullptr;
      const size_t want = (size_t)((used + overflow_bytes) * 1.25) + (1 << 20);
      overflow_bytes = 0;
      cap = 0;
      if (cudaMalloc(reinterpret_cast<void**>(&base), want + shift) == cudaSuccess) { cap = want; base += shift; }
      else cudaGetLastError();
    }
    return 0;
  }
  void destroy() {
    for (void* p : overflow) cudaFree(p);
    overflow.clear();
    if (base) cudaFree(base - shift);
    base = nullptr;
    cap = off = 0;
  }
};

struct Param {
  std::string name;
  int64_t shape[2];
  int ndim;
  int64_t count;
  int64_t offset;
  float* dev;
};

}

using namespace lvsr;

struct lvsr_model {
  lvsr_config cfg;
  int device = 0;
  int E;
  std::vector<Param> params;
  std::map<std::string, int> index;
  float* flat = nullptr;
  int64_t flat_count = 0;
  std::vector<float*> Wcat, bcat;
  float* Wd_cat = nullptr;
  float* Wb1 = nullptr;
  float* Wff_cat = nullptr;
  float* bff_cat = nullptr;
  float* FF = nullptr;
  std::vector<float*> Wcat_hi, Wcat_lo;
  float *Wp_hi = nullptr, *Wp_lo = nullptr;
  bool use_tc = true;
  float v_bias = 0.f;
  unsigned* status = nullptr;
  bool force_stepwise = false;
  long long dec_fallbacks = 0;
  int32_t dec_plan[16] = {0};
  int att_cs = 0;
  int32_t enc_plan[LVSR_MAX_LAYERS][16] = {};
  int32_t pre_plan[2] = {0, 0};
  bool finalized = false;
  long long* lm_off = nullptr;
  int *lm_label = nullptr, *lm_next = nullptr;
  float* lm_weight = nullptr;
  int lm_start = 0;
  lvsr_lm_fusion lm_fusion = {};
  unsigned* lm_status = nullptr;
  Arena ws;
  Arena tws;
  float *opt_velocity = nullptr, *opt_ms_step = nullptr, *opt_ms_dx = nullptr;
  float* opt_scratch = nullptr;
  void* opt_desc = nullptr;
  long long burn_in_left = -1;

  float* P(const std::string& n) const {
    auto it = index.find(n);
    return it == index.end() ? nullptr : params[it->second].dev;
  }
};


namespace lvsr {

static const char* const GEN = "/recognizer/generator";
static const char* const TR = "/recognizer/generator/att_trans";
static const char* const ATT = "/recognizer/generator/att_trans/conv_att";
static const char* const CONT = "/recognizer/generator/att_trans/cont_att";

static inline bool content_attention(const lvsr_model* m) { return m->cfg.attention_type == LVSR_ATT_CONTENT; }
static inline std::string att_base(const lvsr_model* m) { return content_attention(m) ? CONT : ATT; }

static inline std::string enc_base(int l, int dir) {
  char buf[128];
  snprintf(buf, sizeof(buf), "/recognizer/encoder/bidir%d/%s", l, dir ? "backward" : "forward");
  return buf;
}

static inline PriorParams prior_of(const lvsr_config& c) {
  PriorParams p;
  p.type = c.prior_type;
  p.initial_begin = c.prior_initial_begin;
  p.initial_end = c.prior_initial_end;
  p.min_speed = c.prior_min_speed;
  p.max_speed = c.prior_max_speed;
  p.before = c.prior_before;
  p.after = c.prior_after;
  return p;
}

struct DeviceGuard {
  int prev = -1;
  explicit DeviceGuard(const lvsr_model* m) {
    if (!m) return;
    int cur = 0;
    if (cudaGetDevice(&cur) == cudaSuccess && cur != m->device) {
      prev = cur;
      cudaSetDevice(m->device);
    }
  }
  ~DeviceGuard() { if (prev >= 0) cudaSetDevice(prev); }
};

struct ArenaScope {
  Arena& ws;
  cudaStream_t st;
  ArenaScope(lvsr_model* mm, cudaStream_t s) : ws(mm->ws), st(s) { ws.bind_stream(s); ws.enter(); }
  ArenaScope(Arena& a, cudaStream_t s) : ws(a), st(s) { ws.bind_stream(s); ws.enter(); }
  ~ArenaScope() { ws.leave(st); }
};

static inline int check_ready(lvsr_model* m) {
  LVSR_CHECK(m != nullptr, "null model");
  if (!m->finalized) return lvsr_model_finalize(m);
  return 0;
}

struct LayerTape {
  const float* X;
  float* pre;
  float* hext;
  float* out;
  int T, Tout, Din, D, k;
  long long mstride;
};

int finalize_on_stream(lvsr_model* m, cudaStream_t st, bool synchronise);
int run_encoder(lvsr_model* m, Arena& ws, const float* x, const float* mask, int T, int B, float* attended,
                float* attended_mask, LayerTape* tape, cudaStream_t st);
int projection_gemm(Arena& ws, const float* A, int M, int K, const float* W, const float* W_hi, const float* W_lo, int N,
                    const float* bias, float* out, cudaStream_t st, int* kpad = nullptr);
int readout_merged(lvsr_model* m, int R, const float* states, const float* ctx, float* merged, cudaStream_t st);
ReadoutArgs readout_args(lvsr_model* m, int R, const float* merged);
static inline bool lm_attached(const lvsr_model* m) { return m->lm_off != nullptr; }
LmFst lm_fst(lvsr_model* m);
void lm_fuse(const lvsr_model* m, ReadoutArgs& r, const float* lm_add);
int lm_report(unsigned status);
size_t encoder_ws_bytes(const lvsr_model* m, int T, int B);
size_t cost_ws_bytes(const lvsr_model* m, int Tp, int B, int L);

int search_expand(lvsr_model* m, const float* attended, const float* preprocessed, const float* attended_mask, int Tp,
                  int U, const int* utt_len, const int* row_utt, const int* row_seg, const int* seg_start, int nseg,
                  int R, const float* states, const float* weights, const long long* step, const float* cost_so_far,
                  const float* lm_add, int k, float* wavg, float* new_weights, float* new_energies, int* top_parent,
                  int* top_symbol, float* top_cost, int* top_count, cudaStream_t st);
int search_advance(lvsr_model* m, const float* attended, const float* preprocessed, const float* attended_mask, int Tp,
                   int U, const int* utt_len, int Rn, const int* parent, const long long* symbols, const int* row_utt,
                   const int* row_seg, const int* seg_start, int nseg, const float* states, const float* weights,
                   const long long* step, const float* wavg, const float* new_weights, const float* new_energies,
                   float* n_states, float* n_wavg, float* n_weights, float* n_energies, long long* n_step,
                   cudaStream_t st);

}
```

attention-lvcsr_b200/recognizer.py:

```python
import io
import logging
import tarfile
from collections import OrderedDict

import numpy as np

from . import _lib
from . import bricks as _bricks
from . import lm as _lm
from .search import BeamSearch, CandidateNotFoundError


logger = logging.getLogger(__name__)


class _Variable(object):

    def __init__(self, name):
        self.name = name

    def __repr__(self):
        return self.name


def _ptr(t):
    return None if t is None else t.data_ptr()


LM_DEFAULTS = OrderedDict(weight=0.0, normalize_am_weights=True, normalize_lm_weights=False,
                          normalize_tot_weights=False, am_beta=1.0, no_transition_cost=1e12, type_="fst")


def _lm_config(lm):
    unknown = sorted(set(lm) - set(LM_DEFAULTS) - {"path"})
    if unknown:
        raise TypeError("unknown lm option(s) %s" % unknown)
    out = OrderedDict(LM_DEFAULTS)
    out.update(lm)
    if out["type_"] != "fst":
        raise ValueError("lm type_ %r: only 'fst' exists" % (out["type_"],))
    if not (out["normalize_am_weights"] or out["normalize_lm_weights"] or out["normalize_tot_weights"]):
        logger.warning("Beam search is prone to fail with no log-prob normalization")
    return out


class _Child(object):

    def __init__(self, name, **attrs):
        self.name = name
        self.children = []
        for k, v in attrs.items():
            setattr(self, k, v)


class SpeechRecognizer(object):
    def __init__(self, input_dims, input_num_chars, eos_label, num_phonemes,
                 dim_dec, dims_bidir, enc_transition=None, dec_transition=None,
                 use_states_for_readout=True, attention_type="content_and_conv",
                 criterion=None, bottom=None, lm=None, character_map=None,
                 bidir=True, subsample=None, dims_top=None, prior=None, conv_n=None,
                 post_merge_activation=None, post_merge_dims=None, dim_matcher=None,
                 embed_outputs=True, dim_output_embedding=None, dec_stack=1,
                 conv_num_filters=1, data_prepend_eos=True, energy_normalizer=None,
                 max_decoded_length_scale=1, name="recognizer", device=None, **kwargs):
        def unsupported(what):
            raise NotImplementedError("attention-lvcsr_b200: %s is outside the GPU hot path "
                                      "(SURVEY.md section 8)" % what)
        if attention_type not in _lib.ATTENTION_TYPES:
            unsupported("attention_type=%r" % attention_type)
        if lm and not lm.get("path"):
            unsupported("lm without a path")
        if lm and character_map is None:
            unsupported("lm without a character_map")
        lm = _lm_config(lm) if lm else None
        if not bidir:
            unsupported("unidirectional encoder")
        if dims_top:
            unsupported("dims_top")
        if dec_stack != 1:
            unsupported("dec_stack > 1")
        if criterion is not None and criterion.get("name", "log_likelihood") != "log_likelihood":
            unsupported("criterion %r" % criterion.get("name"))
        if bottom and bottom.get("dims"):
            unsupported("bottom MLP")
        for tr in (enc_transition, dec_transition):
            if tr is not None and getattr(tr, "__name__", type(tr).__name__) != "GatedRecurrent":
                unsupported("transition %r" % tr)
        if post_merge_dims is not None and len(post_merge_dims) != 1:
            unsupported("deep post_merge")

        self.name = name
        self.eos_label = eos_label
        self.data_prepend_eos = data_prepend_eos
        self.character_map = character_map
        self.lm = lm
        self._lm_tables = _lm.load(lm["path"], character_map, int(num_phonemes)) if lm else None
        self.criterion = criterion or dict(name="log_likelihood")
        self.max_decoded_length_scale = max_decoded_length_scale
        self.rec_weights_init = None
        self.initial_states_init = None
        self.weights_init = None
        self.biases_init = None

        act = post_merge_activation if post_merge_activation is not None else _bricks.Tanh()
        if dim_matcher is None:
            dim_matcher = dim_dec
        content = attention_type == "content"
        if conv_n is None and not content:
            raise ValueError("conv_n is required for content_and_conv attention")
        subsample = list(subsample) if subsample else [1] * len(dims_bidir)
        prior = dict(prior) if prior else dict(type="expanding", initial_begin=0, initial_end=10000,
                                               min_speed=0, max_speed=0)
        if content:
            conv_n, conv_num_filters, energy_normalizer, prior = 0, 0, None, None
        self.net = dict(
            num_features=int(input_dims["recordings"]), dims_bidir=[int(d) for d in dims_bidir],
            subsample=[int(k) for k in subsample], dim_dec=int(dim_dec), dim_matcher=int(dim_matcher),
            conv_n=int(conv_n), conv_num_filters=int(conv_num_filters), num_phonemes=int(num_phonemes),
            dim_feedback=(int(dim_dec if dim_output_embedding is None else dim_output_embedding) if embed_outputs
                          else int(num_phonemes) + 1),
            embed_outputs=bool(embed_outputs),
            post_merge_dim=int(post_merge_dims[0]) if post_merge_dims else int(num_phonemes),
            post_merge_activation=act.kind, maxout_pieces=int(getattr(act, "num_pieces", 1)),
            use_states_for_readout=bool(use_states_for_readout),
            energy_normalizer=energy_normalizer or "softmax", prior=prior, attention_type=attention_type)
        if not post_merge_dims:
            self.net["post_merge_activation"] = "identity"
            unsupported("readout without post_merge_dims")

        if content:
            attention = _Child("cont_att")
        else:
            attention = _Child("conv_att", prior=prior, energy_normalizer=self.net["energy_normalizer"])
        transition = _Child("att_trans", attention=attention)
        readout = _Child("readout", emitter=_Child("emitter"), readout=None)
        self.generator = _Child("generator", transition=transition, readout=readout)
        self.encoder = _Child("encoder")
        self.top = _Child("top")
        self.bottom = _Child("bottom")
        self.children = [self.encoder, self.top, self.bottom, self.generator]

        self.inputs = OrderedDict(recordings=_Variable("recordings"))
        self.single_inputs = OrderedDict(recordings=_Variable("recordings"))
        self.inputs_mask = _Variable("recordings_mask")
        self.labels = _Variable("labels")
        self.labels_mask = _Variable("labels_mask")
        self.single_labels = _Variable("labels")
        self.n_steps = _Variable("n_steps")

        self._device = device
        self._handle = None
        self._beam_search = None
        self.beam_size = None
        self._ctor_state = None

    def _torch(self):
        import torch
        if not torch.cuda.is_available():
            raise RuntimeError("attention-lvcsr_b200 needs a CUDA device (no CPU fallback)")
        return torch

    @property
    def device(self):
        torch = self._torch()
        if self._device is None:
            self._device = torch.device("cuda", torch.cuda.current_device())
        return torch.device(self._device)

    def _make_config(self):
        import ctypes as C
        n = self.net
        cfg = _lib.LvsrConfig()
        cfg.num_features = n["num_features"]
        cfg.num_layers = len(n["dims_bidir"])
        for i, (d, k) in enumerate(zip(n["dims_bidir"], n["subsample"])):
            cfg.dims_bidir[i] = d
            cfg.subsample[i] = k
        cfg.dim_dec = n["dim_dec"]
        cfg.dim_matcher = n["dim_matcher"]
        cfg.conv_n = n["conv_n"]
        cfg.conv_num_filters = n["conv_num_filters"]
        cfg.num_phonemes = n["num_phonemes"]
        cfg.dim_feedback = n["dim_feedback"]
        cfg.post_merge_dim = n["post_merge_dim"]
        cfg.maxout_pieces = n["maxout_pieces"]
        cfg.post_merge_activation = _lib.ACTIVATIONS[n["post_merge_activation"]]
        cfg.use_states_for_readout = int(n["use_states_for_readout"])
        cfg.energy_normalizer = _lib.NORMALIZERS[n["energy_normalizer"]]
        cfg.attention_type = _lib.ATTENTION_TYPES[n.get("attention_type", "content_and_conv")]
        p = n["prior"] or {}
        cfg.prior_type = _lib.PRIORS[p.get("type", "expanding")]
        cfg.prior_initial_begin = float(p.get("initial_begin", 0))
        cfg.prior_initial_end = float(p.get("initial_end", 10000))
        cfg.prior_min_speed = float(p.get("min_speed", 0))
        cfg.prior_max_speed = float(p.get("max_speed", 0))
        cfg.prior_before = float(p.get("before", 0))
        cfg.prior_after = float(p.get("after", 0))
        cfg.one_of_n_feedback = 0 if n.get("embed_outputs", True) else 1
        return cfg

    def _require_ready(self):
        if self._handle is None:
            import ctypes as C
            torch = self._torch()
            lib = _lib.load()
            with torch.cuda.device(self.device):
                h = C.c_void_p()
                cfg = self._make_config()
                _lib.check(lib.lvsr_model_create(C.byref(cfg), C.byref(h)))
            self._handle = h
            if self.lm:
                self._attach_lm(lib, h)
        return self._handle

    def _attach_lm(self, lib, h):
        import ctypes as C
        t, o = self._lm_tables, self.lm
        fusion = _lib.LvsrLmFusion(weight=float(o["weight"]), am_beta=float(o["am_beta"]),
                                   no_transition_cost=float(o["no_transition_cost"]),
                                   normalize_am_weights=int(bool(o["normalize_am_weights"])),
                                   normalize_lm_weights=int(bool(o["normalize_lm_weights"])),
                                   normalize_tot_weights=int(bool(o["normalize_tot_weights"])))
        try:
            _lib.check(lib.lvsr_model_set_lm(h, t["num_states"], t["start"], t["offsets"].ctypes.data, len(t["label"]),
                                             t["label"].ctypes.data, t["next"].ctypes.data, t["weight"].ctypes.data,
                                             C.byref(fusion)))
        except Exception:
            lib.lvsr_model_destroy(h)
            self._handle = None
            raise

    def __del__(self):
        try:
            if self._handle is not None:
                _lib.load().lvsr_model_destroy(self._handle)
                self._handle = None
        except Exception:
            pass

    def _stream(self):
        return self._torch().cuda.current_stream(self.device).cuda_stream

    def parameter_shapes(self):
        import ctypes as C
        lib, h = _lib.load(), self._require_ready()
        out = OrderedDict()
        for i in range(lib.lvsr_model_num_params(h)):
            shape = (C.c_int64 * 2)()
            ndim = C.c_int32()
            _lib.check(lib.lvsr_model_param_shape(h, i, shape, C.byref(ndim)))
            out[lib.lvsr_model_param_name(h, i).decode()] = tuple(int(shape[j]) for j in range(ndim.value))
        return out

    def set_parameter_values(self, values):
        lib, h = _lib.load(), self._require_ready()
        shapes = self.parameter_shapes()
        for name, value in values.items():
            if name not in shapes:
                raise KeyError("unknown parameter %s" % name)
            arr = np.ascontiguousarray(value, dtype=np.float32)
            if tuple(arr.shape) != shapes[name]:
                raise ValueError("parameter %s: expected shape %s, got %s" % (name, shapes[name], arr.shape))
            _lib.check(lib.lvsr_model_set_param(h, name.encode(), arr.ctypes.data, arr.size))
        _lib.check(lib.lvsr_model_finalize(h))

    def get_parameter_values(self):
        lib, h = _lib.load(), self._require_ready()
        out = OrderedDict()
        for name, shape in self.parameter_shapes().items():
            arr = np.empty(shape, dtype=np.float32)
            _lib.check(lib.lvsr_model_get_param(h, name.encode(), arr.ctypes.data, arr.size))
            out[name] = arr
        return out

    def initialize(self, seed=1):
        w_init = self.weights_init or _bricks.IsotropicGaussian(0.01)
        b_init = self.biases_init or _bricks.Constant(0.0)
        rec_init = self.rec_weights_init or w_init
        h0_init = self.initial_states_init or _bricks.Constant(0.0)
        rng = np.random.RandomState(seed)
        values = OrderedDict()
        for name, shape in self.parameter_shapes().items():
            leaf = name.rsplit(".", 1)[1]
            if leaf == "b":
                v = b_init.generate(rng, shape)
            elif leaf == "state_to_state":
                v = rec_init.generate(rng, shape)
            elif leaf == "state_to_gates":
                d = shape[0]
                v = np.hstack([rec_init.generate(rng, (d, d)), rec_init.generate(rng, (d, d))])
            elif leaf == "initial_state":
                v = h0_init.generate(rng, shape)
            else:
                v = w_init.generate(rng, shape)
            values[name] = np.asarray(v, dtype=np.float32).reshape(shape)
        self.set_parameter_values(values)

    def load_params(self, path):
        data = None
        if tarfile.is_tarfile(path):
            with tarfile.open(path) as tar:
                data = np.load(io.BytesIO(tar.extractfile("_parameters").read()))
        else:
            data = np.load(path)
        values = {k.replace("|", "/"): data[k] for k in data.files}
        shapes = self.parameter_shapes()
        unknown = sorted(set(values) - set(shapes))
        missing = sorted(set(shapes) - set(values))
        if unknown:
            logger.error("unknown parameter names: {}\n".format(unknown))
        if missing:
            logger.error("missing values for parameters: {}\n".format(missing))
        self.set_parameter_values({k: v for k, v in values.items() if k in shapes})
        return dict(unknown=unknown, missing=missing)

    def save_params(self, path):
        buf = io.BytesIO()
        np.savez(buf, **{k.replace("/", "|"): v for k, v in self.get_parameter_values().items()})
        payload = buf.getvalue()
        with tarfile.open(path, "w") as tar:
            info = tarfile.TarInfo("_parameters")
            info.size = len(payload)
            tar.addfile(info, io.BytesIO(payload))

    def __getstate__(self):
        state = dict(self.__dict__)
        for attr in ("_handle", "_beam_search", "_generator_state", "_lm_tables"):
            state.pop(attr, None)
        state["_device"] = None if self._device is None else str(self._device)
        state["_saved_parameters"] = None if self._handle is None else self.get_parameter_values()
        return state

    def __setstate__(self, state):
        saved = state.pop("_saved_parameters", None)
        self.__dict__.update(state)
        self._handle = None
        self._beam_search = None
        lm = self.__dict__.get("lm")
        self.lm = lm
        self._lm_tables = _lm.load(lm["path"], self.character_map, self.net["num_phonemes"]) if lm else None
        if saved is not None:
            try:
                self.set_parameter_values(saved)
            except RuntimeError:
                self._pending_parameters = saved

    def _dev(self, a, dtype=None):
        torch = self._torch()
        if a is None:
            return None
        if isinstance(a, torch.Tensor):
            t = a.to(self.device)
        else:
            t = torch.as_tensor(np.ascontiguousarray(a), device=self.device)
        if dtype is not None and t.dtype != dtype:
            t = t.to(dtype)
        return t.contiguous()

    def launch_status(self):
        import ctypes as C
        lib, h = _lib.load(), self._require_ready()
        st, fb = C.c_int32(), C.c_int64()
        _lib.check(lib.lvsr_model_status(h, C.byref(st), C.byref(fb)))
        return int(st.value), int(fb.value)

    def decoder_plan(self):
        import ctypes as C
        lib, h = _lib.load(), self._require_ready()
        out = (C.c_int32 * 16)()
        _lib.check(lib.lvsr_model_decoder_plan(h, out))
        plan = {k: int(out[i]) for i, k in enumerate(_lib.PLAN_SLOTS)}
        plan["ran"] = bool(plan["ran"])
        plan["kernel"] = _lib.PLAN_KERNELS[plan["kernel"]]
        return plan

    def _encoder_plan_row(self, layer):
        import ctypes as C
        lib, h = _lib.load(), self._require_ready()
        out = (C.c_int32 * 16)()
        _lib.check(lib.lvsr_model_encoder_plan(h, int(layer), out))
        plan = {k: int(out[i]) for i, k in enumerate(_lib.ENC_PLAN_SLOTS)}
        for k in ("proj", "wgrad", "dx"):
            plan[k] = _lib.ENC_PATHS[plan[k]]
        plan["bigru"] = _lib.ENC_BIGRU_KERNELS[plan["bigru"]]
        plan["tape"] = bool(plan["tape"])
        return plan

    def encoder_plan(self):
        return [self._encoder_plan_row(l) for l in range(len(self.net["dims_bidir"]))]

    def preprocess_plan(self):
        plan = self._encoder_plan_row(-1)
        return {"proj": plan["proj"], "kpad": plan["kpad"]}

    def encoded_length(self, T):
        return int(_lib.load().lvsr_encoded_length(self._require_ready(), int(T)))

    @property
    def dim_encoded(self):
        return 2 * self.net["dims_bidir"][-1]

    def encode(self, recordings, recordings_mask=None):
        torch = self._torch()
        lib, h = _lib.load(), self._require_ready()
        x = self._dev(recordings, torch.float32)
        m = self._dev(recordings_mask, torch.float32)
        if x.dim() != 3:
            raise ValueError("encode: recordings [T,B,F] expected")
        T, B, F = x.shape
        if F != self.net["num_features"]:
            raise ValueError("expected %d features, got %d" % (self.net["num_features"], F))
        if m is not None and tuple(m.shape) != (T, B):
            raise ValueError("encode: recordings_mask must be [%d, %d], got %s" % (T, B, tuple(m.shape)))
        Tp = self.encoded_length(T)
        att = torch.empty((Tp, B, self.dim_encoded), dtype=torch.float32, device=self.device)
        attm = torch.empty((Tp, B), dtype=torch.float32, device=self.device)
        _lib.check(lib.lvsr_encoder_forward(h, _ptr(x), _ptr(m), T, B, _ptr(att), _ptr(attm), self._stream()))
        return att, attm

    def preprocess(self, attended):
        torch = self._torch()
        lib, h = _lib.load(), self._require_ready()
        Tp, U, _ = attended.shape
        out = torch.empty((Tp, U, self.net["dim_matcher"]), dtype=torch.float32, device=self.device)
        _lib.check(lib.lvsr_preprocess(h, _ptr(attended), Tp, U, _ptr(out), self._stream()))
        return out

    def _check_labels(self, labels):
        if isinstance(labels, np.ndarray) and labels.size:
            lo, hi = int(labels.min()), int(labels.max())
            if lo < 0 or hi >= self.net["num_phonemes"]:
                raise ValueError("labels must lie in [0, %d): got %d..%d" % (self.net["num_phonemes"], lo, hi))

    def cost_matrix(self, labels, labels_mask, attended, attended_mask, return_all=False):
        torch = self._torch()
        lib, h = _lib.load(), self._require_ready()
        self._check_labels(labels)
        y = self._dev(labels, torch.int64)
        ym = self._dev(labels_mask, torch.float32)
        att = self._dev(attended, torch.float32)
        attm = self._dev(attended_mask, torch.float32)
        if y.dim() != 2 or att.dim() != 3 or attm.dim() != 2:
            raise ValueError("cost_matrix: labels [L,B], attended [T',B,E], attended_mask [T',B] expected")
        L, B = y.shape
        Tp = att.shape[0]
        if L < 1 or B < 1 or Tp < 1:
            raise ValueError("cost_matrix: empty labels or attended sequence")
        if tuple(att.shape) != (Tp, B, self.dim_encoded):
            raise ValueError("cost_matrix: attended must be [%d, %d, %d], got %s" % (Tp, B, self.dim_encoded, tuple(att.shape)))
        if tuple(attm.shape) != (Tp, B):
            raise ValueError("cost_matrix: attended_mask must be [%d, %d], got %s" % (Tp, B, tuple(attm.shape)))
        if ym is not None and tuple(ym.shape) != (L, B):
            raise ValueError("cost_matrix: labels_mask must be [%d, %d], got %s" % (L, B, tuple(ym.shape)))
        costs = torch.empty((L, B), dtype=torch.float32, device=self.device)
        extra = {}
        if return_all:
            extra = dict(weights=torch.empty((L, B, Tp), dtype=torch.float32, device=self.device),
                         energies=torch.empty((L, B, Tp), dtype=torch.float32, device=self.device),
                         states=torch.empty((L, B, self.net["dim_dec"]), dtype=torch.float32, device=self.device),
                         weighted_averages=torch.empty((L, B, self.dim_encoded), dtype=torch.float32,
                                                       device=self.device))
        _lib.check(lib.lvsr_cost_matrix(
            h, _ptr(att), _ptr(attm), Tp, B, _ptr(y), _ptr(ym), L, _ptr(costs),
            _ptr(extra.get("weights")), _ptr(extra.get("energies")), _ptr(extra.get("states")),
            _ptr(extra.get("weighted_averages")), self._stream()))
        if return_all:
            extra["costs"] = costs
            return extra
        return costs

    def cost(self, recordings, recordings_mask, labels, labels_mask):
        lib, h = _lib.load(), self._require_ready()
        x = np.ascontiguousarray(recordings, dtype=np.float32)
        m = None if recordings_mask is None else np.ascontiguousarray(recordings_mask, dtype=np.float32)
        y = np.ascontiguousarray(labels, dtype=np.int64)
        self._check_labels(y)
        ym = None if labels_mask is None else np.ascontiguousarray(labels_mask, dtype=np.float32)
        if x.ndim != 3 or y.ndim != 2:
            raise ValueError("cost: recordings [T,B,F] and labels [L,B] expected")
        T, B, F = x.shape
        L = y.shape[0]
        if F != self.net["num_features"]:
            raise ValueError("expected %d features, got %d" % (self.net["num_features"], F))
        if T < 1 or B < 1 or L < 1:
            raise ValueError("cost: empty batch")
        if m is not None and m.shape != (T, B):
            raise ValueError("cost: recordings_mask must be [%d, %d], got %s" % (T, B, m.shape))
        if y.shape != (L, B):
            raise ValueError("cost: labels must be [L, %d], got %s" % (B, y.shape))
        if ym is not None and ym.shape != (L, B):
            raise ValueError("cost: labels_mask must be [%d, %d], got %s" % (L, B, ym.shape))
        costs = np.empty((L, B), dtype=np.float32)
        torch = self._torch()
        with torch.cuda.device(self.device):
            _lib.check(lib.lvsr_recognizer_cost_host(
                h, x.ctypes.data, None if m is None else m.ctypes.data, y.ctypes.data,
                None if ym is None else ym.ctypes.data, T, B, L, costs.ctypes.data, self._stream()))
        return costs

    def analyze(self, inputs, groundtruth, prediction=None):
        rec = np.asarray(dict(inputs)["recordings"], dtype=np.float32)[:, None, :]
        labels = np.asarray(groundtruth if prediction is None else prediction, dtype=np.int64)[:, None]
        att, attm = self.encode(rec, np.ones(rec.shape[:2], dtype=np.float32))
        r = self.cost_matrix(labels, None, att, attm, return_all=True)
        return [r["costs"][:, 0].cpu().numpy(), r["weights"][:, 0, :].cpu().numpy(),
                r["energies"][:, 0, :].cpu().numpy()]

    def init_beam_search(self, beam_size):
        if self._beam_search is not None and self.beam_size == beam_size:
            return
        self.beam_size = beam_size
        self._beam_search = BeamSearch(beam_size, self)
        self._beam_search.compile()

    def beam_search(self, inputs, **kwargs):
        self.init_beam_search(self.beam_size)
        inputs = dict(inputs)
        rec = np.asarray(inputs.pop("recordings"), dtype=np.float32)
        if inputs:
            raise Exception("Unknown inputs passed to beam search: {}".format(list(inputs.keys())))
        max_length = int(rec.shape[0] / self.max_decoded_length_scale)
        return self._beam_search.search({"recordings": rec[:, None, :]}, self.eos_label, max_length,
                                        ignore_first_eol=self.data_prepend_eos, **kwargs)

    def beam_search_many(self, inputs_list, **kwargs):
        self.init_beam_search(self.beam_size)
        recs = []
        for inputs in inputs_list:
            inputs = dict(inputs)
            recs.append(np.asarray(inputs.pop("recordings"), dtype=np.float32))
            if inputs:
                raise Exception("Unknown inputs passed to beam search: {}".format(list(inputs.keys())))
        max_lengths = [int(x.shape[0] / self.max_decoded_length_scale) for x in recs]
        return self._beam_search.search_many(recs, self.eos_label, max_lengths,
                                             ignore_first_eol=self.data_prepend_eos, **kwargs)

    def generate(self, recordings, recordings_mask=None, n_steps=None, sample=True, seed=None):
        if self.lm:
            raise NotImplementedError("attention-lvcsr_b200: generate / sample with a language model")
        torch = self._torch()
        att, attm = self.encode(recordings, recordings_mask)
        B, Tp = att.shape[1], att.shape[0]
        if n_steps is None:
            n_steps = int(np.asarray(recordings).shape[0] / self.max_decoded_length_scale)
        ctx = dict(attended=att, attended_mask=attm, preprocessed=self.preprocess(att))
        st = self._initial_states(Tp, B)
        gen = None
        if sample:
            gen = torch.Generator(device=self.device)
            gen.manual_seed(1 if seed is None else int(seed))
        outs, costs, states, weights = [], [], [], []
        for _ in range(int(n_steps)):
            neglogp = self._logprobs(ctx, st)
            if sample:
                y = torch.multinomial(torch.exp(-neglogp), 1, generator=gen)[:, 0]
            else:
                y = neglogp.argmin(dim=1)
            costs.append(neglogp.gather(1, y[:, None])[:, 0])
            st = self._next_states(ctx, st, y)
            outs.append(y)
            states.append(st["states"])
            weights.append(st["weights"])
        return dict(outputs=torch.stack(outs).cpu().numpy(), costs=torch.stack(costs).cpu().numpy(),
                    states=torch.stack(states).cpu().numpy(), weights=torch.stack(weights).cpu().numpy())

    def sample(self, inputs, n_steps=None, seed=None):
        rec = np.asarray(dict(inputs)["recordings"], dtype=np.float32)[:, None, :]
        if n_steps is None:
            n_steps = int(rec.shape[0] / self.max_decoded_length_scale)
        return self.generate(rec, None, n_steps=n_steps, sample=True, seed=seed)["outputs"]

    def get_generate_graph(self, use_mask=True, n_steps=None):
        def run(recordings, recordings_mask=None, n_steps=n_steps, **kw):
            return self.generate(recordings, recordings_mask if use_mask else None, n_steps=n_steps, **kw)
        return run

    def get_cost_graph(self, batch=True, prediction=None, prediction_mask=None):
        if batch:
            return lambda recordings, recordings_mask, labels, labels_mask: self.cost(recordings, recordings_mask, labels, labels_mask)
        return lambda recordings, labels: self.analyze({"recordings": recordings}, labels)[0]

    def _initial_states(self, Tp, R):
        torch = self._torch()
        lib, h = _lib.load(), self._require_ready()
        dev = self.device
        st = OrderedDict(
            states=torch.empty((R, self.net["dim_dec"]), dtype=torch.float32, device=dev),
            outputs=torch.empty((R,), dtype=torch.int64, device=dev),
            weighted_averages=torch.empty((R, self.dim_encoded), dtype=torch.float32, device=dev),
            weights=torch.empty((R, Tp), dtype=torch.float32, device=dev),
            energies=torch.empty((R, Tp), dtype=torch.float32, device=dev),
            step=torch.empty((R,), dtype=torch.int64, device=dev))
        _lib.check(lib.lvsr_initial_states(h, Tp, R, _ptr(st["states"]), _ptr(st["outputs"]),
                                           _ptr(st["weighted_averages"]), _ptr(st["weights"]),
                                           _ptr(st["energies"]), _ptr(st["step"]), self._stream()))
        return st

    def _lm_initial_states(self, R):
        torch = self._torch()
        lib, h = _lib.load(), self._require_ready()
        st = OrderedDict(lm_states=torch.empty((R, _lib.LM_MAX_STATES), dtype=torch.int32, device=self.device),
                         lm_weights=torch.empty((R, _lib.LM_MAX_STATES), dtype=torch.float64, device=self.device),
                         lm_add=torch.empty((R, self.net["num_phonemes"]), dtype=torch.float32, device=self.device))
        _lib.check(lib.lvsr_lm_initial_states(h, R, _ptr(st["lm_states"]), _ptr(st["lm_weights"]), _ptr(st["lm_add"]),
                                              self._stream()))
        return st

    def _lm_next_states(self, st, outputs):
        torch = self._torch()
        lib, h = _lib.load(), self._require_ready()
        y = self._dev(outputs, torch.int64)
        s, w = self._dev(st["lm_states"], torch.int32), self._dev(st["lm_weights"], torch.float64)
        R = s.shape[0]
        nxt = OrderedDict(lm_states=torch.empty_like(s), lm_weights=torch.empty_like(w),
                          lm_add=torch.empty((R, self.net["num_phonemes"]), dtype=torch.float32, device=self.device))
        _lib.check(lib.lvsr_lm_next_states(h, R, _ptr(s), _ptr(w), _ptr(y), _ptr(nxt["lm_states"]),
                                           _ptr(nxt["lm_weights"]), _ptr(nxt["lm_add"]), self._stream()))
        return nxt

    def _row_utt(self, contexts, R):
        torch = self._torch()
        U = contexts["attended"].shape[1]
        ru = contexts.get("row_utt")
        if ru is None:
            if U == R:
                return None
            if U != 1:
                raise ValueError("contexts hold %d utterances for %d rows: pass row_utt" % (U, R))
            ru = torch.zeros((R,), dtype=torch.int32, device=self.device)
        return self._dev(ru, torch.int32)

    def _logprobs(self, contexts, st):
        torch = self._torch()
        lib, h = _lib.load(), self._require_ready()
        att = contexts["attended"]
        Tp, U, _ = att.shape
        R = st["states"].shape[0]
        ru = self._row_utt(contexts, R)
        out = torch.empty((R, self.net["num_phonemes"]), dtype=torch.float32, device=self.device)
        _lib.check(lib.lvsr_logprobs(h, _ptr(att), _ptr(contexts.get("preprocessed")), _ptr(contexts["attended_mask"]),
                                     Tp, U, _ptr(ru), R, _ptr(st["states"].contiguous()),
                                     _ptr(st["weights"].contiguous()), _ptr(st["step"].contiguous()), _ptr(out),
                                     self._stream()))
        return out

    def _next_states(self, contexts, st, outputs):
        torch = self._torch()
        lib, h = _lib.load(), self._require_ready()
        att = contexts["attended"]
        Tp, U, _ = att.shape
        R = st["states"].shape[0]
        ru = self._row_utt(contexts, R)
        y = self._dev(outputs, torch.int64)
        nxt = OrderedDict(
            states=torch.empty_like(st["states"]), outputs=y,
            weighted_averages=torch.empty((R, self.dim_encoded), dtype=torch.float32, device=self.device),
            weights=torch.empty((R, Tp), dtype=torch.float32, device=self.device),
            energies=torch.empty((R, Tp), dtype=torch.float32, device=self.device),
            step=torch.empty((R,), dtype=torch.int64, device=self.device))
        _lib.check(lib.lvsr_next_states(
            h, _ptr(att), _ptr(contexts.get("preprocessed")), _ptr(contexts["attended_mask"]), Tp, U, _ptr(ru), R,
            _ptr(st["states"].contiguous()), _ptr(st["weights"].contiguous()), _ptr(st["step"].contiguous()),
            _ptr(y), _ptr(nxt["states"]), _ptr(nxt["weighted_averages"]), _ptr(nxt["weights"]),
            _ptr(nxt["energies"]), _ptr(nxt["step"]), self._stream()))
        return nxt
```

include/lvsr_b200.h:

```cpp
#ifndef LVSR_B200_H
#define LVSR_B200_H

#include <stdint.h>

#ifdef __cplusplus
extern "C" {
#endif

typedef struct lvsr_model lvsr_model;

enum { LVSR_MAX_LAYERS = 8 };
enum { LVSR_NORM_SOFTMAX = 0, LVSR_NORM_LOGISTIC = 1, LVSR_NORM_RELU = 2 };
enum { LVSR_ACT_MAXOUT = 0, LVSR_ACT_RELU = 1, LVSR_ACT_TANH = 2, LVSR_ACT_IDENTITY = 3 };
enum { LVSR_PRIOR_EXPANDING = 0, LVSR_PRIOR_WINDOW_MEAN = 1, LVSR_PRIOR_WINDOW_MEDIAN = 2 };
enum { LVSR_ATT_CONTENT_AND_CONV = 0, LVSR_ATT_CONTENT = 1 };

typedef struct {
  int32_t num_features;
  int32_t num_layers;
  int32_t dims_bidir[LVSR_MAX_LAYERS];
  int32_t subsample[LVSR_MAX_LAYERS];
  int32_t dim_dec;
  int32_t dim_matcher;
  int32_t conv_n;
  int32_t conv_num_filters;
  int32_t num_phonemes;
  int32_t dim_feedback;
  int32_t post_merge_dim;
  int32_t maxout_pieces;
  int32_t post_merge_activation;
  int32_t use_states_for_readout;
  int32_t energy_normalizer;
  int32_t prior_type;
  double prior_initial_begin, prior_initial_end, prior_min_speed, prior_max_speed;
  double prior_before, prior_after;
  int32_t one_of_n_feedback;
  int32_t attention_type;
} lvsr_config;

const char* lvsr_last_error(void);
int lvsr_version(void);

int lvsr_model_create(const lvsr_config* cfg, lvsr_model** out);
int lvsr_model_destroy(lvsr_model* m);

int lvsr_model_num_params(const lvsr_model* m);
const char* lvsr_model_param_name(const lvsr_model* m, int index);
int lvsr_model_param_shape(const lvsr_model* m, int index, int64_t shape[2], int32_t* ndim);
int lvsr_model_set_param(lvsr_model* m, const char* name, const float* values_host, int64_t count);
int lvsr_model_get_param(const lvsr_model* m, const char* name, float* values_host, int64_t count);
int64_t lvsr_model_flat_size(const lvsr_model* m);
int lvsr_model_param_offset(const lvsr_model* m, int index, int64_t* offset, int64_t* count);
float* lvsr_model_flat_params(lvsr_model* m);
int lvsr_model_finalize(lvsr_model* m);
int lvsr_model_status(lvsr_model* m, int32_t* launch_status, int64_t* stepwise_fallbacks);
enum {
  LVSR_PLAN_RAN = 0,
  LVSR_PLAN_KERNEL = 1,
  LVSR_PLAN_CS = 2,
  LVSR_PLAN_GRID = 3,
  LVSR_PLAN_NISL = 4,
  LVSR_PLAN_NRG = 5,
  LVSR_PLAN_NCG = 6,
  LVSR_PLAN_NC1 = 7,
  LVSR_PLAN_NC2 = 8,
  LVSR_PLAN_NC3 = 9,
  LVSR_PLAN_TC_CAP = 10,
  LVSR_PLAN_WH_ROWS = 11,
  LVSR_PLAN_RED_ALIAS = 12,
  LVSR_PLAN_ATT_CS = 13,
  LVSR_PLAN_MAX_CLUSTERS = 14
};
enum { LVSR_PLAN_STEPWISE = 0, LVSR_PLAN_DEC_SCAN = 1, LVSR_PLAN_DEC_SCAN_COMPACT = 2, LVSR_PLAN_DEC_CONTENT = 3 };
int lvsr_model_decoder_plan(const lvsr_model* m, int32_t out[16]);
enum {
  LVSR_ENC_PROJ = 0,
  LVSR_ENC_KPAD = 1,
  LVSR_ENC_BIGRU = 2,
  LVSR_ENC_TAPE = 3,
  LVSR_ENC_RB = 4,
  LVSR_ENC_CS = 5,
  LVSR_ENC_CLUSTERS = 6,
  LVSR_ENC_RESIDENT = 7,
  LVSR_ENC_WAVES = 8,
  LVSR_ENC_T = 9,
  LVSR_ENC_BWD_CS = 10,
  LVSR_ENC_WGRAD = 11,
  LVSR_ENC_WGRAD_SPLITS = 12,
  LVSR_ENC_WGRAD_KPAD = 13,
  LVSR_ENC_DX = 14
};
enum { LVSR_ENC_PATH_NONE = 0, LVSR_ENC_PATH_TC = 1, LVSR_ENC_PATH_FFMA = 2 };
enum { LVSR_ENC_BIGRU_NONE = 0, LVSR_ENC_BIGRU_FFMA = 1, LVSR_ENC_BIGRU_MMA = 2 };
int lvsr_model_encoder_plan(const lvsr_model* m, int32_t layer, int32_t out[16]);

int lvsr_encoded_length(const lvsr_model* m, int32_t T);
int lvsr_encoded_dim(const lvsr_model* m);
int lvsr_encoder_forward(lvsr_model* m, const float* recordings_dev, const float* mask_dev,
                         int32_t T, int32_t B, float* attended_dev, float* attended_mask_dev,
                         void* stream);

int lvsr_preprocess(lvsr_model* m, const float* attended_dev, int32_t Tp, int32_t U,
                    float* preprocessed_dev, void* stream);

int lvsr_cost_matrix(lvsr_model* m, const float* attended_dev, const float* attended_mask_dev,
                     int32_t Tp, int32_t B, const int64_t* labels_dev, const float* labels_mask_dev,
                     int32_t L, float* costs_dev, float* weights_dev, float* energies_dev,
                     float* states_dev, float* weighted_averages_dev, void* stream);

int lvsr_initial_states(lvsr_model* m, int32_t Tp, int32_t R, float* states_dev, int64_t* outputs_dev,
                        float* weighted_averages_dev, float* weights_dev, float* energies_dev,
                        int64_t* step_dev, void* stream);
int lvsr_logprobs(lvsr_model* m, const float* attended_dev, const float* preprocessed_dev,
                  const float* attended_mask_dev, int32_t Tp, int32_t U, const int32_t* row_utt_dev,
                  int32_t R, const float* states_dev, const float* weights_dev, const int64_t* step_dev,
                  float* neg_logprobs_dev, void* stream);
int lvsr_next_states(lvsr_model* m, const float* attended_dev, const float* preprocessed_dev,
                     const float* attended_mask_dev, int32_t Tp, int32_t U, const int32_t* row_utt_dev,
                     int32_t R, const float* states_dev, const float* weights_dev, const int64_t* step_dev,
                     const int64_t* outputs_dev, float* next_states_dev, float* next_weighted_averages_dev,
                     float* next_weights_dev, float* next_energies_dev, int64_t* next_step_dev,
                     void* stream);

typedef int32_t (*lvsr_validate_fn)(void* validate_user, int32_t utt, const int64_t* tokens, int32_t length);
typedef struct lvsr_search_result lvsr_search_result;
int lvsr_beam_search_many(lvsr_model* m, const float* attended_dev, const float* preprocessed_dev,
                          const float* attended_mask_dev, int32_t Tp, int32_t U, const int32_t* utt_len_host,
                          const int32_t* max_length_host, int32_t beam_size, int32_t eol_symbol,
                          int32_t ignore_first_eol, double char_discount, double round_to_inf,
                          int32_t stop_on_optimistic, lvsr_validate_fn validate, void* validate_user,
                          lvsr_search_result** result, void* stream);
int lvsr_search_result_count(const lvsr_search_result* r, int32_t utt);
int lvsr_search_result_length(const lvsr_search_result* r, int32_t utt, int32_t j);
int lvsr_search_result_get(const lvsr_search_result* r, int32_t utt, int32_t j, int64_t* tokens, float* costs);
int lvsr_search_result_destroy(lvsr_search_result* r);

enum { LVSR_LM_MAX_STATES = 7 };
typedef struct {
  double weight;
  double am_beta;
  double no_transition_cost;
  int32_t normalize_am_weights;
  int32_t normalize_lm_weights;
  int32_t normalize_tot_weights;
} lvsr_lm_fusion;
int lvsr_model_set_lm(lvsr_model* m, int32_t num_states, int32_t start, const int64_t* arc_offsets_host, int64_t num_arcs,
                      const int32_t* arc_label_host, const int32_t* arc_next_host, const float* arc_weight_host,
                      const lvsr_lm_fusion* fusion);
int lvsr_model_clear_lm(lvsr_model* m);
int lvsr_lm_initial_states(lvsr_model* m, int32_t R, int32_t* states_dev, double* weights_dev, float* add_dev,
                           void* stream);
int lvsr_lm_next_states(lvsr_model* m, int32_t R, const int32_t* states_dev, const double* weights_dev,
                        const int64_t* outputs_dev, int32_t* next_states_dev, double* next_weights_dev,
                        float* next_add_dev, void* stream);

int lvsr_recognizer_cost_host(lvsr_model* m, const float* recordings_host, const float* mask_host,
                              const int64_t* labels_host, const float* labels_mask_host,
                              int32_t T, int32_t B, int32_t L, float* costs_host, void* stream);

typedef struct {
  float gradient_threshold;
  int32_t use_momentum;
  float scale, momentum;
  int32_t use_adadelta;
  float decay_rate, epsilon;
  float max_norm;
  int32_t burn_in_steps;
  float decay;
} lvsr_train_config;
int lvsr_train_cost_and_grads(lvsr_model* m, const float* recordings_dev, const float* mask_dev,
                              const int64_t* labels_dev, const float* labels_mask_dev, int32_t T, int32_t B,
                              int32_t L, float gscale, float* cost_dev, float* grads_dev, void* stream);
int lvsr_train_apply_updates(lvsr_model* m, float* grads_dev, float gscale, const lvsr_train_config* tc,
                             void* stream);
int lvsr_train_gradient_norm(lvsr_model* m, float* norm_host);
int lvsr_train_reset(lvsr_model* m);

int64_t lvsr_launch_count(int reset);

int lvsr_profile_enable(int on);
int lvsr_profile_read(const char* kernel_class, double* total_ms, int64_t* count);

#ifdef __cplusplus
}
#endif
#endif
```

Before: 3.570 million.

## Add fp16x3 split-operand wgmma path with per-row exponents and persistent tiles

Adds an fp16 head/tail operand split with per-row and per-column exponent scaling, so the encoder and preprocess projection GEMMs can use m64n128k16 f16 wgmma instead of tf32x3. This doubles K per instruction and halves operand bytes. The TC kernel also becomes persistent, looping over tiles with a grid capped at the SM count, and weights are packed into a single allocation. The cost is an extra row-split kernel for activations and fp16 range and precision handling through exponent rescaling, which risks accuracy differences compared with tf32x3.

```diff
diff --git a/attention-lvcsr_b200/_lib.py b/attention-lvcsr_b200/_lib.py
--- a/attention-lvcsr_b200/_lib.py
+++ b/attention-lvcsr_b200/_lib.py
@@ -13,8 +13,9 @@
               "att_cs", "max_clusters")
 PLAN_KERNELS = ("stepwise", "dec_scan", "dec_scan<COMPACT>", "dec_content")
 ENC_PLAN_SLOTS = ("proj", "kpad", "bigru", "tape", "rb", "cs", "clusters", "resident", "waves", "T", "bwd_cs", "wgrad",
-                  "wgrad_splits", "wgrad_kpad", "dx")
+                  "wgrad_splits", "wgrad_kpad", "dx", "operands")
 ENC_PATHS = (None, "tc", "ffma")
+ENC_OPERANDS = (None, "tf32x3", "f16x3")
 ENC_BIGRU_KERNELS = (None, "ffma", "mma")
 
 
diff --git a/attention-lvcsr_b200/csrc/api.cu b/attention-lvcsr_b200/csrc/api.cu
--- a/attention-lvcsr_b200/csrc/api.cu
+++ b/attention-lvcsr_b200/csrc/api.cu
@@ -362,10 +362,8 @@
   if (m->flat) cudaFree(m->flat);
   for (float* p : m->Wcat) if (p) cudaFree(p);
   for (float* p : m->bcat) if (p) cudaFree(p);
-  for (float* p : m->Wcat_hi) if (p) cudaFree(p);
-  for (float* p : m->Wcat_lo) if (p) cudaFree(p);
-  if (m->Wp_hi) cudaFree(m->Wp_hi);
-  if (m->Wp_lo) cudaFree(m->Wp_lo);
+  for (TcWeights& t : m->Wcat_tc) if (t.mem) cudaFree(t.mem);
+  if (m->Wp_tc.mem) cudaFree(m->Wp_tc.mem);
   if (m->Wd_cat) cudaFree(m->Wd_cat);
   if (m->Wb1) cudaFree(m->Wb1);
   if (m->Wff_cat) cudaFree(m->Wff_cat);
@@ -408,6 +406,7 @@
   if (layer < 0) {
     out[LVSR_ENC_PROJ] = m->pre_plan[0];
     out[LVSR_ENC_KPAD] = m->pre_plan[1];
+    out[LVSR_ENC_OPERANDS] = m->pre_plan[2];
   }
   return 0;
 }
@@ -532,6 +531,27 @@
 }
 
 namespace lvsr {
+static int pack_tc_weights(TcWeights& tw, const float* W, int K, int N, cudaStream_t st) {
+  if (!tw.mem) {
+    if (gemm_f16_supported(128, N, K)) {
+      const size_t plane = (size_t)N * K * sizeof(__half);
+      LVSR_CUDA_OK(cudaMalloc(&tw.mem, 2 * plane + (size_t)N * sizeof(int)));
+      tw.head = static_cast<__half*>(tw.mem);
+      tw.tail = reinterpret_cast<__half*>(static_cast<char*>(tw.mem) + plane);
+      tw.ew = reinterpret_cast<int*>(static_cast<char*>(tw.mem) + 2 * plane);
+    } else if (gemm_tc_supported(128, N, K)) {
+      const size_t plane = (size_t)N * gemm_tc_kpad(K);
+      LVSR_CUDA_OK(cudaMalloc(&tw.mem, 2 * plane * sizeof(float)));
+      tw.hi = static_cast<float*>(tw.mem);
+      tw.lo = tw.hi + plane;
+    } else {
+      return 0;
+    }
+  }
+  if (tw.head) return split_weight_f16(W, K, N, tw.head, tw.tail, tw.ew, st);
+  return split_weight_tf32(W, K, N, tw.hi, tw.lo, st);
+}
+
 int finalize_on_stream(lvsr_model* m, cudaStream_t st, bool synchronise) {
   const lvsr_config& c = m->cfg;
   if (m->Wcat.empty()) {
@@ -578,34 +598,13 @@
   if (int rc = copy_cols(m->bff_cat, 3 * C, 2 * C, m->P(g + "/fork/fork_inputs.b"), 1, C, st)) return rc;
   m->use_tc = getenv("LVSR_NO_TC_GEMM") == nullptr;
   if (m->use_tc) {
-    if (m->Wcat_hi.empty()) {
-      int dk = c.num_features;
-      for (int l = 0; l < c.num_layers; ++l) {
-        const int D = c.dims_bidir[l];
-        float *h = nullptr, *lo = nullptr;
-        if (gemm_tc_supported(128, 6 * D, dk)) {
-          LVSR_CUDA_OK(cudaMalloc(reinterpret_cast<void**>(&h), (size_t)gemm_tc_kpad(dk) * 6 * D * sizeof(float)));
-          LVSR_CUDA_OK(cudaMalloc(reinterpret_cast<void**>(&lo), (size_t)gemm_tc_kpad(dk) * 6 * D * sizeof(float)));
-        }
-        m->Wcat_hi.push_back(h);
-        m->Wcat_lo.push_back(lo);
-        dk = 2 * D;
-      }
-      if (gemm_tc_supported(128, c.dim_matcher, m->E)) {
-        LVSR_CUDA_OK(cudaMalloc(reinterpret_cast<void**>(&m->Wp_hi), (size_t)gemm_tc_kpad(m->E) * c.dim_matcher * sizeof(float)));
-        LVSR_CUDA_OK(cudaMalloc(reinterpret_cast<void**>(&m->Wp_lo), (size_t)gemm_tc_kpad(m->E) * c.dim_matcher * sizeof(float)));
-      }
-    }
+    m->Wcat_tc.resize(c.num_layers);
     int dk = c.num_features;
     for (int l = 0; l < c.num_layers; ++l) {
-      const int D = c.dims_bidir[l];
-      if (m->Wcat_hi[l])
-        if (int rc = split_weight_tf32(m->Wcat[l], dk, 6 * D, m->Wcat_hi[l], m->Wcat_lo[l], st)) return rc;
-      dk = 2 * D;
-    }
-    if (m->Wp_hi)
-      if (int rc = split_weight_tf32(m->P(att_base(m) + "/preprocess.W"), m->E, c.dim_matcher, m->Wp_hi, m->Wp_lo, st))
-        return rc;
+      if (int rc = pack_tc_weights(m->Wcat_tc[l], m->Wcat[l], dk, 6 * c.dims_bidir[l], st)) return rc;
+      dk = 2 * c.dims_bidir[l];
+    }
+    if (int rc = pack_tc_weights(m->Wp_tc, m->P(att_base(m) + "/preprocess.W"), m->E, c.dim_matcher, st)) return rc;
   }
   if (c.one_of_n_feedback) {
     if (int rc = add_bias_rows(m->FF, m->Wff_cat, m->bff_cat, V + 1, 3 * C, st)) return rc;
@@ -623,16 +622,25 @@
   return 0;
 }
 
-int projection_gemm(Arena& ws, const float* A, int M, int K, const float* W, const float* W_hi, const float* W_lo, int N,
-                    const float* bias, float* out, cudaStream_t st, int* kpad) {
-  if (W_hi && gemm_tc_supported(M, N, K)) {
+int projection_gemm(Arena& ws, const float* A, int M, int K, const float* W, const TcWeights* tw, int N,
+                    const float* bias, float* out, cudaStream_t st, int* kpad, int* operands) {
+  const bool f16 = tw && tw->head && gemm_f16_supported(M, N, K);
+  const bool tf32 = tw && tw->hi && gemm_tc_supported(M, N, K);
+  if (f16 || tf32) {
     float* a_hi = ws.f32((size_t)M * gemm_tc_kpad(K));
     float* a_lo = ws.f32((size_t)M * gemm_tc_kpad(K));
-    LVSR_CHECK(a_hi && a_lo, "out of device memory (tf32 split scratch)");
+    LVSR_CHECK(a_hi && a_lo, "out of device memory (tensor-core split scratch)");
     if (kpad) *kpad = gemm_tc_kpad(K);
-    return gemm_tc(A, a_hi, a_lo, M, K, W_hi, W_lo, N, bias, out, N, st);
+    if (operands) *operands = f16 ? LVSR_ENC_OPS_F16X3 : LVSR_ENC_OPS_TF32X3;
+    if (f16) {
+      __half* a_head = reinterpret_cast<__half*>(a_hi);
+      return gemm_f16(A, a_head, a_head + (size_t)M * K, reinterpret_cast<int*>(a_lo), M, K, tw->head, tw->tail, tw->ew,
+                      N, bias, out, N, st);
+    }
+    return gemm_tc(A, a_hi, a_lo, M, K, tw->hi, tw->lo, N, bias, out, N, st);
   }
   if (kpad) *kpad = 0;
+  if (operands) *operands = LVSR_ENC_OPS_NONE;
   return gemm_bias(make_gemm(A, M, K, W, N, bias, out), st);
 }
 
@@ -643,8 +651,10 @@
   int Tl = T, din = c.num_features;
   long long mstride = B;
   int kcum = 1;
-  for (int l = 0; l < c.num_layers; ++l)
+  for (int l = 0; l < c.num_layers; ++l) {
     for (int s = LVSR_ENC_PROJ; s <= LVSR_ENC_T; ++s) m->enc_plan[l][s] = 0;
+    m->enc_plan[l][LVSR_ENC_OPERANDS] = 0;
+  }
   for (int l = 0; l < c.num_layers; ++l) {
     const int D = c.dims_bidir[l], k = c.subsample[l];
     const int rows = Tl * B, Tout = ceil_div(Tl, k);
@@ -653,12 +663,13 @@
     LVSR_CHECK(pre && (hext || !tape), "out of device memory (encoder pre-activations)");
     const size_t mark = ws.off;
     int32_t* plan = m->enc_plan[l];
-    int kpad = 0;
-    if (int rc = projection_gemm(ws, cur, rows, din, m->Wcat[l], m->use_tc ? m->Wcat_hi[l] : nullptr,
-                                 m->use_tc ? m->Wcat_lo[l] : nullptr, 6 * D, m->bcat[l], pre, st, &kpad))
+    int kpad = 0, operands = 0;
+    if (int rc = projection_gemm(ws, cur, rows, din, m->Wcat[l], m->use_tc ? &m->Wcat_tc[l] : nullptr, 6 * D, m->bcat[l],
+                                 pre, st, &kpad, &operands))
       return rc;
     plan[LVSR_ENC_PROJ] = kpad ? LVSR_ENC_PATH_TC : LVSR_ENC_PATH_FFMA;
     plan[LVSR_ENC_KPAD] = kpad;
+    plan[LVSR_ENC_OPERANDS] = operands;
     if (ws.off <= ws.cap) ws.off = mark;
     float* out = (l == c.num_layers - 1) ? attended : ws.f32((size_t)Tout * B * 2 * D);
     LVSR_CHECK(out, "out of device memory (encoder layer output)");
@@ -720,14 +731,15 @@
   LVSR_CHECK(attended && out && Tp > 0 && U > 0, "preprocess: bad arguments");
   cudaStream_t st = static_cast<cudaStream_t>(stream);
   ArenaScope scope(m, st);
-  int kpad = 0;
-  m->pre_plan[0] = m->pre_plan[1] = 0;
+  int kpad = 0, operands = 0;
+  m->pre_plan[0] = m->pre_plan[1] = m->pre_plan[2] = 0;
   if (int rc = projection_gemm(m->ws, attended, Tp * U, m->E, m->P(att_base(m) + "/preprocess.W"),
-                               m->use_tc ? m->Wp_hi : nullptr, m->Wp_lo, m->cfg.dim_matcher,
-                               m->P(att_base(m) + "/preprocess.b"), out, st, &kpad))
+                               m->use_tc ? &m->Wp_tc : nullptr, m->cfg.dim_matcher, m->P(att_base(m) + "/preprocess.b"),
+                               out, st, &kpad, &operands))
     return rc;
   m->pre_plan[0] = kpad ? LVSR_ENC_PATH_TC : LVSR_ENC_PATH_FFMA;
   m->pre_plan[1] = kpad;
+  m->pre_plan[2] = operands;
   return 0;
 }
 
diff --git a/attention-lvcsr_b200/csrc/gemm_tc.cu b/attention-lvcsr_b200/csrc/gemm_tc.cu
--- a/attention-lvcsr_b200/csrc/gemm_tc.cu
+++ b/attention-lvcsr_b200/csrc/gemm_tc.cu
@@ -1,4 +1,5 @@
 #include <cuda.h>
+#include <cuda_fp16.h>
 
 #include "kernels.h"
 
@@ -7,9 +8,10 @@
 namespace {
 
 constexpr int TC_BM = 128, TC_BN = 128, TC_BK = 32;
+constexpr int TC_BK_F16 = 64;
 constexpr int TC_THREADS = 384;
 constexpr int TC_STAGES = 3;
-constexpr uint32_t TC_TILE_BYTES = TC_BM * TC_BK * sizeof(float);
+constexpr uint32_t TC_TILE_BYTES = TC_BM * 128;
 constexpr uint32_t TC_STAGE_BYTES = 4 * TC_TILE_BYTES;
 constexpr size_t TC_SMEM = (size_t)TC_STAGES * TC_STAGE_BYTES + 1024  + 256 ;
 
@@ -66,30 +68,50 @@
 
 #define LVSR_ACC8(d, i) \
   "+f"(d[i]), "+f"(d[i + 1]), "+f"(d[i + 2]), "+f"(d[i + 3]), "+f"(d[i + 4]), "+f"(d[i + 5]), "+f"(d[i + 6]), "+f"(d[i + 7])
-__device__ __forceinline__ void wgmma_tf32_n128(float (&d)[64], uint64_t desc_a, uint64_t desc_b, uint32_t scale_d) {
-  asm volatile(
-      "{\n\t.reg .pred p;\n\t"
-      "setp.ne.b32 p, %66, 0;\n\t"
-      "wgmma.mma_async.sync.aligned.m64n128k8.f32.tf32.tf32 {"
-      "%0, %1, %2, %3, %4, %5, %6, %7, %8, %9, %10, %11, %12, %13, %14, %15, "
-      "%16, %17, %18, %19, %20, %21, %22, %23, %24, %25, %26, %27, %28, %29, %30, %31, "
-      "%32, %33, %34, %35, %36, %37, %38, %39, %40, %41, %42, %43, %44, %45, %46, %47, "
-      "%48, %49, %50, %51, %52, %53, %54, %55, %56, %57, %58, %59, %60, %61, %62, %63"
-      "}, %64, %65, p, 1, 1;\n\t}\n"
-      : LVSR_ACC8(d, 0), LVSR_ACC8(d, 8), LVSR_ACC8(d, 16), LVSR_ACC8(d, 24),
-        LVSR_ACC8(d, 32), LVSR_ACC8(d, 40), LVSR_ACC8(d, 48), LVSR_ACC8(d, 56)
-      : "l"(desc_a), "l"(desc_b), "r"(scale_d));
-}
+#define LVSR_ACC64 "{"                                                                        \
+  "%0, %1, %2, %3, %4, %5, %6, %7, %8, %9, %10, %11, %12, %13, %14, %15, "                    \
+  "%16, %17, %18, %19, %20, %21, %22, %23, %24, %25, %26, %27, %28, %29, %30, %31, "          \
+  "%32, %33, %34, %35, %36, %37, %38, %39, %40, %41, %42, %43, %44, %45, %46, %47, "          \
+  "%48, %49, %50, %51, %52, %53, %54, %55, %56, %57, %58, %59, %60, %61, %62, %63}"
+template <bool F16>
+__device__ __forceinline__ void wgmma_n128(float (&d)[64], uint64_t desc_a, uint64_t desc_b, uint32_t scale_d) {
+  if constexpr (F16) {
+    asm volatile(
+        "{\n\t.reg .pred p;\n\t"
+        "setp.ne.b32 p, %66, 0;\n\t"
+        "wgmma.mma_async.sync.aligned.m64n128k16.f32.f16.f16 " LVSR_ACC64 ", %64, %65, p, 1, 1, 0, 0;\n\t}\n"
+        : LVSR_ACC8(d, 0), LVSR_ACC8(d, 8), LVSR_ACC8(d, 16), LVSR_ACC8(d, 24),
+          LVSR_ACC8(d, 32), LVSR_ACC8(d, 40), LVSR_ACC8(d, 48), LVSR_ACC8(d, 56)
+        : "l"(desc_a), "l"(desc_b), "r"(scale_d));
+  } else {
+    asm volatile(
+        "{\n\t.reg .pred p;\n\t"
+        "setp.ne.b32 p, %66, 0;\n\t"
+        "wgmma.mma_async.sync.aligned.m64n128k8.f32.tf32.tf32 " LVSR_ACC64 ", %64, %65, p, 1, 1;\n\t}\n"
+        : LVSR_ACC8(d, 0), LVSR_ACC8(d, 8), LVSR_ACC8(d, 16), LVSR_ACC8(d, 24),
+          LVSR_ACC8(d, 32), LVSR_ACC8(d, 40), LVSR_ACC8(d, 48), LVSR_ACC8(d, 56)
+        : "l"(desc_a), "l"(desc_b), "r"(scale_d));
+  }
+}
+#undef LVSR_ACC64
 #undef LVSR_ACC8
 
 struct TcGemmParams {
   float* C;
   const float* bias;
+  const int* ea;
+  const int* eb;
   int M, N, K, ldc;
+  int tiles_n, tiles_m, tiles;
   int kb_per_split;
   long long c_split_stride;
 };
 
+__device__ __forceinline__ float unscale(float x, int e) {
+  return (unsigned)(e + 126) <= 252u ? x * __uint_as_float((uint32_t)(127 - e) << 23) : ldexpf(x, -e);
+}
+
+template <bool F16>
 __global__ void __launch_bounds__(TC_THREADS, 1)
 gemm_tc_kernel(const __grid_constant__ CUtensorMap map_a_hi, const __grid_constant__ CUtensorMap map_a_lo,
                const __grid_constant__ CUtensorMap map_b_hi, const __grid_constant__ CUtensorMap map_b_lo,
@@ -97,13 +119,11 @@
   extern __shared__ uint8_t smem_raw[];
   uint8_t* tiles = reinterpret_cast<uint8_t*>((reinterpret_cast<uintptr_t>(smem_raw) + 1023) & ~(uintptr_t)1023);
   constexpr int NACC = TC_BN / 2;
+  constexpr int BK = F16 ? TC_BK_F16 : TC_BK;
   unsigned long long* bars = reinterpret_cast<unsigned long long*>(tiles + (size_t)TC_STAGES * TC_STAGE_BYTES);
 
   const int wg = threadIdx.x >> 7, t = threadIdx.x & 127;
-  const int n0 = blockIdx.x * TC_BN, m0 = blockIdx.y * TC_BM;
-  const int kb0 = blockIdx.z * p.kb_per_split;
-  const int nkb = min(p.kb_per_split, p.K / TC_BK - kb0);
-  p.C += (long long)blockIdx.z * p.c_split_stride;
+  const int total_kb = p.K / BK;
 
   if (threadIdx.x == 0) {
     for (int s = 0; s < TC_STAGES; ++s) {
@@ -116,62 +136,160 @@
 
   if (wg == 0) {
     if (t == 0) {
-      for (int kb = 0; kb < nkb; ++kb) {
-        const int s = kb % TC_STAGES;
-        const uint32_t ph = (uint32_t)((kb / TC_STAGES) & 1);
-        bar_wait(smem_addr(&bars[TC_STAGES + s]), ph ^ 1u);
-        const uint32_t full = smem_addr(&bars[s]);
-        bar_expect_tx(full, TC_STAGE_BYTES);
-        const uint32_t base = smem_addr(tiles + (size_t)s * TC_STAGE_BYTES);
-        tma_load_2d(base + 0 * TC_TILE_BYTES, &map_a_hi, (kb0 + kb) * TC_BK, m0, full);
-        tma_load_2d(base + 1 * TC_TILE_BYTES, &map_a_lo, (kb0 + kb) * TC_BK, m0, full);
-        tma_load_2d(base + 2 * TC_TILE_BYTES, &map_b_hi, (kb0 + kb) * TC_BK, n0, full);
-        tma_load_2d(base + 3 * TC_TILE_BYTES, &map_b_lo, (kb0 + kb) * TC_BK, n0, full);
+      uint32_t it = 0;
+      for (int tile = blockIdx.x; tile < p.tiles; tile += gridDim.x) {
+        const int n0 = (tile % p.tiles_n) * TC_BN, m0 = (tile / p.tiles_n % p.tiles_m) * TC_BM;
+        const int kb0 = tile / (p.tiles_n * p.tiles_m) * p.kb_per_split;
+        const int nkb = min(p.kb_per_split, total_kb - kb0);
+        for (int kb = 0; kb < nkb; ++kb, ++it) {
+          const uint32_t s = it % TC_STAGES;
+          const uint32_t ph = (it / TC_STAGES) & 1u;
+          bar_wait(smem_addr(&bars[TC_STAGES + s]), ph ^ 1u);
+          const uint32_t full = smem_addr(&bars[s]);
+          bar_expect_tx(full, TC_STAGE_BYTES);
+          const uint32_t base = smem_addr(tiles + (size_t)s * TC_STAGE_BYTES);
+          tma_load_2d(base + 0 * TC_TILE_BYTES, &map_a_hi, (kb0 + kb) * BK, m0, full);
+          tma_load_2d(base + 1 * TC_TILE_BYTES, &map_a_lo, (kb0 + kb) * BK, m0, full);
+          tma_load_2d(base + 2 * TC_TILE_BYTES, &map_b_hi, (kb0 + kb) * BK, n0, full);
+          tma_load_2d(base + 3 * TC_TILE_BYTES, &map_b_lo, (kb0 + kb) * BK, n0, full);
+        }
       }
     }
     return;
   }
 
   const uint32_t a_off = (uint32_t)(wg - 1) * 64 * 128;
-  float acc[NACC];
-#pragma unroll
-  for (int i = 0; i < NACC; ++i) acc[i] = 0.f;
-  for (int kb = 0; kb < nkb; ++kb) {
-    const int s = kb % TC_STAGES;
-    bar_wait(smem_addr(&bars[s]), (uint32_t)((kb / TC_STAGES) & 1));
-    const uint32_t base = smem_addr(tiles + (size_t)s * TC_STAGE_BYTES);
-    const uint64_t da_hi = make_smem_desc(base + 0 * TC_TILE_BYTES + a_off), da_lo = make_smem_desc(base + 1 * TC_TILE_BYTES + a_off);
-    const uint64_t db_hi = make_smem_desc(base + 2 * TC_TILE_BYTES), db_lo = make_smem_desc(base + 3 * TC_TILE_BYTES);
-    wgmma_fence();
-#pragma unroll
-    for (int k = 0; k < 4; ++k) {
-      const uint64_t adv = (uint64_t)(k * 2);
-      wgmma_tf32_n128(acc, da_lo + adv, db_hi + adv, 1u);
-      wgmma_tf32_n128(acc, da_hi + adv, db_lo + adv, 1u);
-      wgmma_tf32_n128(acc, da_hi + adv, db_hi + adv, 1u);
-    }
-    wgmma_commit();
-    wgmma_wait<1>();
+  const int warp = t >> 5, lane = t & 31;
+  uint32_t it = 0;
+  for (int tile = blockIdx.x; tile < p.tiles; tile += gridDim.x) {
+    const int n0 = (tile % p.tiles_n) * TC_BN, m0 = (tile / p.tiles_n % p.tiles_m) * TC_BM;
+    const int split = tile / (p.tiles_n * p.tiles_m);
+    const int nkb = min(p.kb_per_split, total_kb - split * p.kb_per_split);
+    float acc[NACC];
+#pragma unroll
+    for (int i = 0; i < NACC; ++i) acc[i] = 0.f;
+    for (int kb = 0; kb < nkb; ++kb, ++it) {
+      const uint32_t s = it % TC_STAGES;
+      bar_wait(smem_addr(&bars[s]), (it / TC_STAGES) & 1u);
+      const uint32_t base = smem_addr(tiles + (size_t)s * TC_STAGE_BYTES);
+      const uint64_t da_hi = make_smem_desc(base + 0 * TC_TILE_BYTES + a_off), da_lo = make_smem_desc(base + 1 * TC_TILE_BYTES + a_off);
+      const uint64_t db_hi = make_smem_desc(base + 2 * TC_TILE_BYTES), db_lo = make_smem_desc(base + 3 * TC_TILE_BYTES);
+      wgmma_fence();
+#pragma unroll
+      for (int k = 0; k < 4; ++k) {
+        const uint64_t adv = (uint64_t)(k * 2);
+        wgmma_n128<F16>(acc, da_lo + adv, db_hi + adv, 1u);
+        wgmma_n128<F16>(acc, da_hi + adv, db_lo + adv, 1u);
+        wgmma_n128<F16>(acc, da_hi + adv, db_hi + adv, 1u);
+      }
+      wgmma_commit();
+      wgmma_wait<1>();
+      acc_fence(acc);
+      if (kb > 0 && t == 0) bar_arrive(smem_addr(&bars[TC_STAGES + (it - 1) % TC_STAGES]));
+    }
+    wgmma_wait<0>();
     acc_fence(acc);
-    if (kb > 0 && t == 0) bar_arrive(smem_addr(&bars[TC_STAGES + (kb - 1) % TC_STAGES]));
-  }
-  wgmma_wait<0>();
-  acc_fence(acc);
-
-  const int warp = t >> 5, lane = t & 31;
-  const int r0 = m0 + (wg - 1) * 64 + warp * 16 + (lane >> 2);
-  const int cbase = n0 + 2 * (lane & 3);
-#pragma unroll
-  for (int j = 0; j < TC_BN / 8; ++j) {
-    const int col = cbase + 8 * j;
-    float2 b = make_float2(0.f, 0.f);
-    if (p.bias) b = __ldg(reinterpret_cast<const float2*>(p.bias + col));
-#pragma unroll
-    for (int h = 0; h < 2; ++h) {
-      const int row = r0 + 8 * h;
-      const float x = acc[4 * j + 2 * h], y = acc[4 * j + 2 * h + 1];
-      if (row < p.M) *reinterpret_cast<float2*>(p.C + (long long)row * p.ldc + col) = make_float2(x + b.x, y + b.y);
-    }
+    if (t == 0) bar_arrive(smem_addr(&bars[TC_STAGES + (it - 1) % TC_STAGES]));
+
+    float* C = p.C + (long long)split * p.c_split_stride;
+    const int r0 = m0 + (wg - 1) * 64 + warp * 16 + (lane >> 2);
+    const int cbase = n0 + 2 * (lane & 3);
+    float2 bias[TC_BN / 8];
+    int2 eb[TC_BN / 8];
+    int ea[2] = {0, 0};
+#pragma unroll
+    for (int j = 0; j < TC_BN / 8; ++j) {
+      bias[j] = p.bias ? __ldg(reinterpret_cast<const float2*>(p.bias + cbase + 8 * j)) : make_float2(0.f, 0.f);
+      eb[j] = F16 ? __ldg(reinterpret_cast<const int2*>(p.eb + cbase + 8 * j)) : make_int2(0, 0);
+    }
+    if constexpr (F16) {
+#pragma unroll
+      for (int h = 0; h < 2; ++h) ea[h] = r0 + 8 * h < p.M ? __ldg(p.ea + r0 + 8 * h) : 0;
+    }
+#pragma unroll
+    for (int j = 0; j < TC_BN / 8; ++j) {
+      const int col = cbase + 8 * j;
+#pragma unroll
+      for (int h = 0; h < 2; ++h) {
+        const int row = r0 + 8 * h;
+        float x = acc[4 * j + 2 * h], y = acc[4 * j + 2 * h + 1];
+        if constexpr (F16) {
+          x = unscale(x, ea[h] + eb[j].x);
+          y = unscale(y, ea[h] + eb[j].y);
+        }
+        if (row < p.M) *reinterpret_cast<float2*>(C + (long long)row * p.ldc + col) = make_float2(x + bias[j].x, y + bias[j].y);
+      }
+    }
+  }
+}
+
+__device__ __forceinline__ int f16_range_exponent(float max_abs) {
+  if (max_abs == 0.f) return 0;
+  return min(140 - (int)((__float_as_uint(max_abs) >> 23) & 0xFFu), 127);
+}
+__device__ __forceinline__ float exp2_int(int e) { return __uint_as_float((uint32_t)(e + 127) << 23); }
+__device__ __forceinline__ void split_f16(float y, __half& head, __half& tail) {
+  head = __float2half_rn(y);
+  tail = __float2half_rn(y - __half2float(head));
+}
+
+__global__ void split_rows_f16_kernel(const float* __restrict__ x, __half* __restrict__ head, __half* __restrict__ tail,
+                                      int* __restrict__ e, long long M, int K) {
+  const long long r = (long long)blockIdx.x * (blockDim.x >> 5) + (threadIdx.x >> 5);
+  const int lane = threadIdx.x & 31;
+  if (r >= M) return;
+  const float2* row = reinterpret_cast<const float2*>(x + r * K);
+  float mx = 0.f;
+  for (int i = lane; i < K / 2; i += 32) {
+    const float2 v = row[i];
+    mx = fmaxf(mx, fmaxf(fabsf(v.x), fabsf(v.y)));
+  }
+#pragma unroll
+  for (int o = 16; o > 0; o >>= 1) mx = fmaxf(mx, __shfl_xor_sync(0xffffffffu, mx, o));
+  const int er = f16_range_exponent(mx);
+  const float s = exp2_int(er);
+  if (lane == 0) e[r] = er;
+  __half2* h2 = reinterpret_cast<__half2*>(head + r * K);
+  __half2* t2 = reinterpret_cast<__half2*>(tail + r * K);
+  for (int i = lane; i < K / 2; i += 32) {
+    const float2 v = row[i];
+    __half hx, hy, tx, ty;
+    split_f16(v.x * s, hx, tx);
+    split_f16(v.y * s, hy, ty);
+    h2[i] = __halves2half2(hx, hy);
+    t2[i] = __halves2half2(tx, ty);
+  }
+}
+
+__global__ void transpose_split_f16_kernel(const float* __restrict__ W, __half* __restrict__ head, __half* __restrict__ tail,
+                                           int* __restrict__ e, int K, int N) {
+  __shared__ float tile[32][33];
+  __shared__ float scale[32];
+  const int n0 = blockIdx.x * 32, tx = threadIdx.x, ty = threadIdx.y;
+  const int n = n0 + tx;
+  float mx = 0.f;
+  if (n < N)
+    for (int k = ty; k < K; k += 8) mx = fmaxf(mx, fabsf(W[(long long)k * N + n]));
+  tile[ty][tx] = mx;
+  __syncthreads();
+  if (ty == 0) {
+    for (int i = 1; i < 8; ++i) mx = fmaxf(mx, tile[i][tx]);
+    const int en = f16_range_exponent(mx);
+    if (n < N) e[n] = en;
+    scale[tx] = exp2_int(en);
+  }
+  __syncthreads();
+  for (int k0 = 0; k0 < K; k0 += 32) {
+    for (int i = ty; i < 32; i += 8) {
+      const int k = k0 + i;
+      tile[i][tx] = (k < K && n < N) ? W[(long long)k * N + n] * scale[tx] : 0.f;
+    }
+    __syncthreads();
+    for (int i = ty; i < 32; i += 8) {
+      const int nn = n0 + i, k = k0 + tx;
+      if (nn < N && k < K) split_f16(tile[tx][i], head[(long long)nn * K + k], tail[(long long)nn * K + k]);
+    }
+    __syncthreads();
   }
 }
 
@@ -245,15 +363,52 @@
   return 0;
 }
 
-int make_map(CUtensorMap* map, const float* ptr, long long rows, int K, int box_rows = TC_BM) {
+int make_map(CUtensorMap* map, const void* ptr, long long rows, int K, bool f16) {
+  const size_t esize = f16 ? sizeof(__half) : sizeof(float);
   cuuint64_t dims[2] = {(cuuint64_t)K, (cuuint64_t)rows};
-  cuuint64_t strides[1] = {(cuuint64_t)K * sizeof(float)};
-  cuuint32_t box[2] = {(cuuint32_t)TC_BK, (cuuint32_t)box_rows};
+  cuuint64_t strides[1] = {(cuuint64_t)K * esize};
+  cuuint32_t box[2] = {(cuuint32_t)(128 / esize), (cuuint32_t)TC_BM};
   cuuint32_t estr[2] = {1, 1};
-  CUresult r = g_encode(map, CU_TENSOR_MAP_DATA_TYPE_FLOAT32, 2, const_cast<float*>(ptr), dims, strides, box, estr,
-                        CU_TENSOR_MAP_INTERLEAVE_NONE, CU_TENSOR_MAP_SWIZZLE_128B, CU_TENSOR_MAP_L2_PROMOTION_L2_128B,
-                        CU_TENSOR_MAP_FLOAT_OOB_FILL_NONE);
+  CUresult r = g_encode(map, f16 ? CU_TENSOR_MAP_DATA_TYPE_FLOAT16 : CU_TENSOR_MAP_DATA_TYPE_FLOAT32, 2,
+                        const_cast<void*>(ptr), dims, strides, box, estr, CU_TENSOR_MAP_INTERLEAVE_NONE,
+                        CU_TENSOR_MAP_SWIZZLE_128B, CU_TENSOR_MAP_L2_PROMOTION_L2_128B, CU_TENSOR_MAP_FLOAT_OOB_FILL_NONE);
   LVSR_CHECK(r == CUDA_SUCCESS, "cuTensorMapEncodeTiled failed (%d)", (int)r);
+  return 0;
+}
+
+template <bool F16>
+int launch_tc(const void* A_hi, const void* A_lo, const int* ea, int M, const void* B_hi, const void* B_lo, const int* eb,
+              int N, int K, const float* bias, float* C, int ldc, int splits, long long split_stride, cudaStream_t stream) {
+  ProfScope prof("gemm", stream);
+  constexpr int BK = F16 ? TC_BK_F16 : TC_BK;
+  LVSR_CHECK(M >= 1 && N % TC_BN == 0 && K % BK == 0 && K >= BK && splits >= 1,
+             "gemm_tc: unsupported shape M=%d N=%d K=%d (%s operands)", M, N, K, F16 ? "fp16" : "tf32");
+  if (int rc = get_encode()) return rc;
+  CUtensorMap ma_hi, ma_lo, mb_hi, mb_lo;
+  if (int rc = make_map(&ma_hi, A_hi, M, K, F16)) return rc;
+  if (int rc = make_map(&ma_lo, A_lo, M, K, F16)) return rc;
+  if (int rc = make_map(&mb_hi, B_hi, N, K, F16)) return rc;
+  if (int rc = make_map(&mb_lo, B_lo, N, K, F16)) return rc;
+  static bool configured[LVSR_MAX_DEVICES] = {false};
+  const int dev = current_device();
+  if (!configured[dev]) {
+    LVSR_CUDA_OK(cudaFuncSetAttribute(gemm_tc_kernel<F16>, cudaFuncAttributeMaxDynamicSharedMemorySize, (int)TC_SMEM));
+    configured[dev] = true;
+  }
+  const int total_kb = K / BK;
+  splits = std::min(splits, total_kb);
+  TcGemmParams p;
+  p.C = C; p.bias = bias; p.ea = ea; p.eb = eb; p.M = M; p.N = N; p.K = K; p.ldc = ldc;
+  p.kb_per_split = ceil_div(total_kb, splits);
+  p.c_split_stride = split_stride;
+  p.tiles_n = N / TC_BN;
+  p.tiles_m = ceil_div(M, TC_BM);
+  const long long tiles = (long long)p.tiles_n * p.tiles_m * ceil_div(total_kb, p.kb_per_split);
+  LVSR_CHECK(tiles <= INT32_MAX, "gemm_tc: too many tiles (M=%d N=%d)", M, N);
+  p.tiles = (int)tiles;
+  const int grid = (int)std::min<long long>(tiles, device_sm_count());
+  gemm_tc_kernel<F16><<<grid, TC_THREADS, TC_SMEM, stream>>>(ma_hi, ma_lo, mb_hi, mb_lo, p);
+  LVSR_LAUNCH_CHECK();
   return 0;
 }
 
@@ -298,30 +453,7 @@
 
 int gemm_tc_presplit(const float* A_hi, const float* A_lo, int M, const float* B_hi, const float* B_lo, int N, int Kpad,
                      const float* bias, float* C, int ldc, int splits, long long split_stride, cudaStream_t stream) {
-  ProfScope prof("gemm", stream);
-  LVSR_CHECK(M >= 1 && N % TC_BN == 0 && Kpad % TC_BK == 0 && Kpad >= TC_BK && splits >= 1, "gemm_tc_presplit: unsupported shape M=%d N=%d K=%d", M, N, Kpad);
-  if (int rc = get_encode()) return rc;
-  CUtensorMap ma_hi, ma_lo, mb_hi, mb_lo;
-  if (int rc = make_map(&ma_hi, A_hi, M, Kpad)) return rc;
-  if (int rc = make_map(&ma_lo, A_lo, M, Kpad)) return rc;
-  if (int rc = make_map(&mb_hi, B_hi, N, Kpad)) return rc;
-  if (int rc = make_map(&mb_lo, B_lo, N, Kpad)) return rc;
-  static bool configured[LVSR_MAX_DEVICES] = {false};
-  const int dev = current_device();
-  if (!configured[dev]) {
-    LVSR_CUDA_OK(cudaFuncSetAttribute(gemm_tc_kernel, cudaFuncAttributeMaxDynamicSharedMemorySize, (int)TC_SMEM));
-    configured[dev] = true;
-  }
-  const int total_kb = Kpad / TC_BK;
-  splits = std::min(splits, total_kb);
-  TcGemmParams p;
-  p.C = C; p.bias = bias; p.M = M; p.N = N; p.K = Kpad; p.ldc = ldc;
-  p.kb_per_split = ceil_div(total_kb, splits);
-  p.c_split_stride = split_stride;
-  dim3 grid(N / TC_BN, ceil_div(M, TC_BM), ceil_div(total_kb, p.kb_per_split));
-  gemm_tc_kernel<<<grid, TC_THREADS, TC_SMEM, stream>>>(ma_hi, ma_lo, mb_hi, mb_lo, p);
-  LVSR_LAUNCH_CHECK();
-  return 0;
+  return launch_tc<false>(A_hi, A_lo, nullptr, M, B_hi, B_lo, nullptr, N, Kpad, bias, C, ldc, splits, split_stride, stream);
 }
 
 int gemm_tc(const float* A, float* A_hi, float* A_lo, int M, int K, const float* Wt_hi, const float* Wt_lo, int N,
@@ -341,4 +473,23 @@
   return gemm_tc_presplit(A_hi, A_lo, M, Wt_hi, Wt_lo, N, Kpad, bias, C, ldc, 1, 0, stream);
 }
 
-}
+bool gemm_f16_supported(int M, int N, int K) { return M >= 1 && N % TC_BN == 0 && K >= TC_BK_F16 && K % TC_BK_F16 == 0; }
+
+int split_weight_f16(const float* W, int K, int N, __half* Wt_head, __half* Wt_tail, int* ew, cudaStream_t stream) {
+  LVSR_CHECK(K % TC_BK_F16 == 0 && K > 0 && N > 0, "split_weight_f16: unsupported shape K=%d N=%d", K, N);
+  transpose_split_f16_kernel<<<ceil_div(N, 32), dim3(32, 8), 0, stream>>>(W, Wt_head, Wt_tail, ew, K, N);
+  LVSR_LAUNCH_CHECK();
+  return 0;
+}
+
+int gemm_f16(const float* A, __half* A_head, __half* A_tail, int* ea, int M, int K, const __half* Wt_head,
+             const __half* Wt_tail, const int* ew, int N, const float* bias, float* C, int ldc, cudaStream_t stream) {
+  LVSR_CHECK(gemm_f16_supported(M, N, K), "gemm_f16: unsupported shape M=%d N=%d K=%d", M, N, K);
+  constexpr int ROWS_PER_BLOCK = 8;
+  split_rows_f16_kernel<<<ceil_div(M, ROWS_PER_BLOCK), 32 * ROWS_PER_BLOCK, 0, stream>>>(
+      A, A_head, A_tail, ea, M, K);
+  LVSR_LAUNCH_CHECK();
+  return launch_tc<true>(A_head, A_tail, ea, M, Wt_head, Wt_tail, ew, N, K, bias, C, ldc, 1, 0, stream);
+}
+
+}
diff --git a/attention-lvcsr_b200/csrc/kernels.h b/attention-lvcsr_b200/csrc/kernels.h
--- a/attention-lvcsr_b200/csrc/kernels.h
+++ b/attention-lvcsr_b200/csrc/kernels.h
@@ -1,4 +1,6 @@
 #pragma once
+#include <cuda_fp16.h>
+
 #include "common.cuh"
 
 namespace lvsr {
@@ -36,6 +38,10 @@
 int gemm_tc_splits_launched(int Kpad, int splits);
 int gemm_tc(const float* A, float* A_hi, float* A_lo, int M, int K, const float* Wt_hi, const float* Wt_lo, int N,
             const float* bias, float* C, int ldc, cudaStream_t stream);
+bool gemm_f16_supported(int M, int N, int K);
+int split_weight_f16(const float* W, int K, int N, __half* Wt_head, __half* Wt_tail, int* ew, cudaStream_t stream);
+int gemm_f16(const float* A, __half* A_head, __half* A_tail, int* ea, int M, int K, const __half* Wt_head,
+             const __half* Wt_tail, const int* ew, int N, const float* bias, float* C, int ldc, cudaStream_t stream);
 
 struct BiGruArgs {
   const float* pre;
diff --git a/attention-lvcsr_b200/csrc/model.h b/attention-lvcsr_b200/csrc/model.h
--- a/attention-lvcsr_b200/csrc/model.h
+++ b/attention-lvcsr_b200/csrc/model.h
@@ -78,6 +78,13 @@
   }
 };
 
+struct TcWeights {
+  void* mem = nullptr;
+  __half *head = nullptr, *tail = nullptr;
+  int* ew = nullptr;
+  float *hi = nullptr, *lo = nullptr;
+};
+
 struct Param {
   std::string name;
   int64_t shape[2];
@@ -105,8 +112,8 @@
   float* Wff_cat = nullptr;
   float* bff_cat = nullptr;
   float* FF = nullptr;
-  std::vector<float*> Wcat_hi, Wcat_lo;
-  float *Wp_hi = nullptr, *Wp_lo = nullptr;
+  std::vector<TcWeights> Wcat_tc;
+  TcWeights Wp_tc;
   bool use_tc = true;
   float v_bias = 0.f;
   unsigned* status = nullptr;
@@ -115,7 +122,7 @@
   int32_t dec_plan[16] = {0};
   int att_cs = 0;
   int32_t enc_plan[LVSR_MAX_LAYERS][16] = {};
-  int32_t pre_plan[2] = {0, 0};
+  int32_t pre_plan[3] = {0, 0, 0};
   bool finalized = false;
   long long* lm_off = nullptr;
   int *lm_label = nullptr, *lm_next = nullptr;
@@ -204,8 +211,8 @@
 int finalize_on_stream(lvsr_model* m, cudaStream_t st, bool synchronise);
 int run_encoder(lvsr_model* m, Arena& ws, const float* x, const float* mask, int T, int B, float* attended,
                 float* attended_mask, LayerTape* tape, cudaStream_t st);
-int projection_gemm(Arena& ws, const float* A, int M, int K, const float* W, const float* W_hi, const float* W_lo, int N,
-                    const float* bias, float* out, cudaStream_t st, int* kpad = nullptr);
+int projection_gemm(Arena& ws, const float* A, int M, int K, const float* W, const TcWeights* tw, int N,
+                    const float* bias, float* out, cudaStream_t st, int* kpad = nullptr, int* operands = nullptr);
 int readout_merged(lvsr_model* m, int R, const float* states, const float* ctx, float* merged, cudaStream_t st);
 ReadoutArgs readout_args(lvsr_model* m, int R, const float* merged);
 static inline bool lm_attached(const lvsr_model* m) { return m->lm_off != nullptr; }
diff --git a/attention-lvcsr_b200/recognizer.py b/attention-lvcsr_b200/recognizer.py
--- a/attention-lvcsr_b200/recognizer.py
+++ b/attention-lvcsr_b200/recognizer.py
@@ -383,6 +383,7 @@
         for k in ("proj", "wgrad", "dx"):
             plan[k] = _lib.ENC_PATHS[plan[k]]
         plan["bigru"] = _lib.ENC_BIGRU_KERNELS[plan["bigru"]]
+        plan["operands"] = _lib.ENC_OPERANDS[plan["operands"]]
         plan["tape"] = bool(plan["tape"])
         return plan
 
diff --git a/include/lvsr_b200.h b/include/lvsr_b200.h
--- a/include/lvsr_b200.h
+++ b/include/lvsr_b200.h
@@ -88,9 +88,11 @@
   LVSR_ENC_WGRAD = 11,
   LVSR_ENC_WGRAD_SPLITS = 12,
   LVSR_ENC_WGRAD_KPAD = 13,
-  LVSR_ENC_DX = 14
+  LVSR_ENC_DX = 14,
+  LVSR_ENC_OPERANDS = 15
 };
 enum { LVSR_ENC_PATH_NONE = 0, LVSR_ENC_PATH_TC = 1, LVSR_ENC_PATH_FFMA = 2 };
+enum { LVSR_ENC_OPS_NONE = 0, LVSR_ENC_OPS_TF32X3 = 1, LVSR_ENC_OPS_F16X3 = 2 };
 enum { LVSR_ENC_BIGRU_NONE = 0, LVSR_ENC_BIGRU_FFMA = 1, LVSR_ENC_BIGRU_MMA = 2 };
 int lvsr_model_encoder_plan(const lvsr_model* m, int32_t layer, int32_t out[16]);
 
```

Result: faster. 3.748 million, median of 6 (+5.0%).
